# JunyiPeng00/wespeaker_hubert

Hardware: AMD Instinct MI355X
Metric: embeddings/sec on 5s 16kHz utts (higher is better)
Workload: dtype f32 (bf16x3 split MFMA, fp32 accumulate)

## Files before the change

wespeaker_hubert_amd/csrc/conv_gemm.hip:

```cpp
#include "gemm_common.h"

namespace wsp {

namespace {

constexpr int BK = 32;
constexpr int LDK = BK + 4;

template <int WM, int WN, int TM, int TN, int AMODE, bool UNI>
__global__ __launch_bounds__(256, 2) void conv_gemm_f32(const ConvGemmArgs p) {
  constexpr int BM = WM * TM * 32;
  constexpr int BN = WN * TN * 32;
  constexpr int AR = BM / 32;
  constexpr int BR = BN / 32;
  static_assert(WM * WN == 4, "4 waves");

  extern __shared__ __attribute__((aligned(16))) float smem[];
  float* As = smem;
  float* Bs = smem + 2 * BM * LDK;

  const int tid = threadIdx.x;
  const int lane = tid & 63;
  const int wave = tid >> 6;
  const int ntiles = p.N / BN;
  const int mtiles = (p.M + BM - 1) / BM;
  const int wg = xcd_remap(blockIdx.x, ntiles * mtiles);
  const int mt = wg / ntiles;
  const int nt = wg - mt * ntiles;
  const int m0 = mt * BM;
  const int n0 = nt * BN;

  const int srow = tid >> 3;
  const int c4 = (tid & 7) * 4;
  ALoader<AR, AMODE, UNI> al;
  al.init(p, m0, srow, 32, c4);
  if (p.gcols) al.a0 += (n0 / p.gcols) * p.gcin;
  const __amdgpu_buffer_rsrc_t rw = make_rsrc(p.w);
  int woff[BR];
#pragma unroll
  for (int i = 0; i < BR; ++i) woff[i] = ((n0 + srow + 32 * i) * p.Kp + c4) * 4;

  f32x4 ra[AR], rb[BR];

  auto load_tile = [&](int k0) {
#pragma unroll
    for (int i = 0; i < BR; ++i) rb[i] = bload4(rw, woff[i] + k0 * 4);
    al.load(k0, ra);
  };

  auto store_tile = [&](int buf) {
    float* a = As + buf * BM * LDK;
    float* b = Bs + buf * BN * LDK;
#pragma unroll
    for (int i = 0; i < AR; ++i)
      *reinterpret_cast<f32x4*>(a + (srow + 32 * i) * LDK + c4) = ra[i];
#pragma unroll
    for (int i = 0; i < BR; ++i)
      *reinterpret_cast<f32x4*>(b + (srow + 32 * i) * LDK + c4) = rb[i];
  };

  const int wm = wave / WN;
  const int wn = wave - wm * WN;
  const int r32 = lane & 31;
  const int h = lane >> 5;

  f32x16 acc[TM][TN];
#pragma unroll
  for (int i = 0; i < TM; ++i)
#pragma unroll
    for (int j = 0; j < TN; ++j)
#pragma unroll
      for (int r = 0; r < 16; ++r) acc[i][j][r] = 0.f;

  const int nk = p.Kp / BK;
  load_tile(0);
  store_tile(0);
  __syncthreads();

  for (int kt = 0; kt < nk; ++kt) {
    const int cur = kt & 1;
    if (kt + 1 < nk) load_tile((kt + 1) * BK);
    const float* a = As + cur * BM * LDK + (wm * TM * 32 + r32) * LDK + h * 16;
    const float* b = Bs + cur * BN * LDK + (wn * TN * 32 + r32) * LDK + h * 16;
#pragma unroll
    for (int q = 0; q < 4; ++q) {
      f32x4 af[TM], bf[TN];
#pragma unroll
      for (int i = 0; i < TM; ++i) af[i] = *reinterpret_cast<const f32x4*>(a + i * 32 * LDK + q * 4);
#pragma unroll
      for (int j = 0; j < TN; ++j) bf[j] = *reinterpret_cast<const f32x4*>(b + j * 32 * LDK + q * 4);
#pragma unroll
      for (int s = 0; s < 4; ++s)
#pragma unroll
        for (int i = 0; i < TM; ++i)
#pragma unroll
          for (int j = 0; j < TN; ++j)
            acc[i][j] = __builtin_amdgcn_mfma_f32_32x32x2f32(af[i][s], bf[j][s], acc[i][j], 0, 0, 0);
    }
    if (kt + 1 < nk) store_tile(cur ^ 1);
    __syncthreads();
  }

  gemm_epilogue<TM, TN>(p, acc, m0, n0, wm, wn, lane);
}

template <int WM, int WN, int TM, int TN, int AMODE, bool UNI>
void launch_k(const ConvGemmArgs& p, hipStream_t s) {
  constexpr int BM = WM * TM * 32, BN = WN * TN * 32;
  const int nwg = ((p.M + BM - 1) / BM) * (p.N / BN);
  const size_t lds = (size_t)2 * (BM + BN) * LDK * sizeof(float);
  hipLaunchKernelGGL((conv_gemm_f32<WM, WN, TM, TN, AMODE, UNI>), dim3(nwg), dim3(256), lds, s, p);
  WSP_HIP(hipGetLastError());
}

template <int WM, int WN, int TM, int TN>
void launch_tile(const ConvGemmArgs& p, hipStream_t s) {
  const bool uni = uniform_ktiles(p);
  if (p.amode == kAAdd) {
    if (uni) launch_k<WM, WN, TM, TN, kAAdd, true>(p, s);
    else launch_k<WM, WN, TM, TN, kAAdd, false>(p, s);
  } else {
    if (uni) launch_k<WM, WN, TM, TN, kACat, true>(p, s);
    else launch_k<WM, WN, TM, TN, kACat, false>(p, s);
  }
}

}

int conv_gemm_tile_for(int N) { return (N % 128 == 0) ? 0 : 1; }

void launch_conv_gemm(const ConvGemmArgs& args, hipStream_t s) {
  const ConvGemmArgs p = normalized(args);
  check_conv_args(p, "conv_gemm");
  WSP_CHECK(!p.colsum, "conv_gemm: column sums are a bf16x3-kernel epilogue");
  WSP_CHECK(!p.conv2d && p.N % 64 == 0, "conv_gemm (f32): 1-D convs with N % 64 == 0 only");
  WSP_CHECK(!p.gcols || p.gcols % 64 == 0, "conv_gemm (f32): grouped columns must be a multiple of 64");
  WSP_CHECK(!p.sc2d && !p.lnmode && !p.gate && !p.seam_h && !p.seam_out,
            "conv_gemm (f32): conv3 + shortcut, the LayerNorm fold, the gated A tail and the seam run on tile family 7");
  if (conv_gemm_tile_for(p.N) == 0 && !p.gcols)
    launch_tile<2, 2, 2, 2>(p, s);
  else
    launch_tile<4, 1, 1, 2>(p, s);
}

}
```

wespeaker_hubert_amd/csrc/conv_gemm_x3.hip:

```cpp
#include "conv_gemm_x3_impl.h"

namespace wsp {

int conv_gemm_x3_block_rows(const ConvGemmArgs& p, int variant) {
  if (p.N % 64 != 0 || (p.gcols && p.gcols % 64 != 0)) return 128;
  if (p.gcols || p.N % 128 != 0) return 128;
  return variant == 3 ? 128 : 256;
}

namespace {
__global__ __launch_bounds__(256) void colsum_mean_kernel(const double* __restrict__ part, int bm, int T, int N,
                                                          float* __restrict__ out, int ldo) {
  const int b = blockIdx.y;
  const int n = blockIdx.x * 256 + threadIdx.x;
  if (n >= N) return;
  const long r0 = (long)b * T, r1 = r0 + T;
  double v = 0.0;
  for (long mt = r0 / bm; mt * bm < r1; ++mt) {
    const int slot = (mt * bm) / T == b ? 0 : 1;
    v += part[((size_t)mt * 2 + slot) * N + n];
  }
  out[(long)b * ldo + n] = (float)(v / (double)T);
}
}

void launch_colsum_mean(const double* part, int block_rows, int T, int B, int N, float* out, int ldo,
                        hipStream_t s) {
  WSP_CHECK(block_rows > 0 && T >= block_rows && B > 0 && N > 0, "colsum_mean: bad shape");
  hipLaunchKernelGGL(colsum_mean_kernel, dim3((N + 255) / 256, B), dim3(256), 0, s, part, block_rows, T, N, out,
                     ldo);
  WSP_HIP(hipGetLastError());
}

bool conv_gemm_x3_gate_ok(const ConvGemmArgs& args, int variant) {
  return variant == 7 && args.gate && x3::g256_gate_supported(normalized(args));
}

bool conv_gemm_x3_seam_ok(const ConvGemmArgs& args, int variant) {
  return variant == 7 && args.seam_h && x3::seam_supported(normalized(args));
}

void launch_conv_gemm_x3(const ConvGemmArgs& args, const void* whi, const void* wlo, int variant,
                         hipStream_t s) {
  const ConvGemmArgs p = normalized(args);
  check_conv_args(p, "conv_gemm_x3");
  if (p.colsum) {
    const int bm = conv_gemm_x3_block_rows(p, variant);
    WSP_CHECK(!p.seg && !p.row_bias && !p.conv2d && p.T >= bm,
              "conv_gemm_x3: column sums need a uniform batch with T >= block rows and no row bias");
  }
  WSP_CHECK(p.Kp % 64 == 0, "conv_gemm_x3: packed K must be a multiple of 64");
  WSP_CHECK(variant >= 3 && variant <= 7, "conv_gemm_x3: tile family must be 3, 4, 5, 6 or 7");
  const __bf16* h = static_cast<const __bf16*>(whi);
  const __bf16* l = static_cast<const __bf16*>(wlo);
  x3::TileFn f;
  if (p.seam_h || p.seam_out) {
    WSP_CHECK(variant == 7 && x3::seam_supported(p),
              "conv_gemm_x3: the seam runs on tile family 7 only (conv_gemm_x3_seam_ok)");
    x3::t_seam(p, h, l, s);
    return;
  }
  WSP_CHECK(!p.lnmode || (variant == 7 && x3::g256_supported(p)),
            "conv_gemm_x3: the LayerNorm fold runs on tile family 7 only");
  WSP_CHECK(!p.sc2d || (variant == 7 && x3::g256_supported(p)),
            "conv_gemm_x3: conv3 + shortcut runs on tile family 7 only (N % 256 == 0, 16-B aligned operands)");
  WSP_CHECK(!p.gate || (variant == 7 && x3::g256_gate_supported(p)),
            "conv_gemm_x3: the gated A tail runs on tile family 7 only (conv_gemm_x3_gate_ok)");
  if (variant == 7 && x3::g256_supported(p)) {
    x3::t_g256(p, h, l, s);
    return;
  }
  if (variant == 7) variant = 6;
  if (p.N % 64 != 0 || (p.gcols && p.gcols % 64 != 0)) {
    f = x3::t_4x1_1x1;
  } else if (p.gcols) {
    f = variant >= 5 ? x3::t_8x1_1x2_sw : x3::t_4x1_1x2;
  } else if (p.N % 128 != 0) {
    f = x3::t_4x1_1x2;
  } else if (variant == 3) {
    f = x3::t_2x2_2x2_sw;
  } else if (variant == 4) {
    f = x3::t_4x2_2x2_sw;
  } else if (p.N % 256 == 0) {
    f = variant == 6 ? x3::t_4x2_2x4_mf16 : x3::t_4x2_2x4_sw1;
  } else {
    f = x3::t_4x2_2x2_sw;
  }
  f(p, h, l, s);
}

}
```

wespeaker_hubert_amd/csrc/conv_gemm_x3_g.h:

```cpp
#pragma once

#include "conv_gemm_x3_impl.h"

namespace wsp {
namespace {

typedef __attribute__((address_space(3))) void lds_void;
constexpr int kGA = 256 * 128, kGW = 256 * 64, kGStage = kGA + 2 * kGW;

__device__ __forceinline__ int g_aslot(int r, int c) { return r * 128 + ((c ^ ((r >> 1) & 5)) << 4); }

__device__ __forceinline__ void g_dma(__amdgpu_buffer_rsrc_t r, unsigned char* lds, int voff) {
  __builtin_amdgcn_raw_ptr_buffer_load_lds(r, (lds_void*)lds, 16, voff, 0, 0, 0);
}

constexpr int kGEpiLd = 132;
constexpr int kGEpiBytes = 8 * 32 * kGEpiLd * 4;
typedef unsigned u32x4 __attribute__((ext_vector_type(4)));

constexpr int kLnMaxParts = 8;
__device__ __forceinline__ void g_ln_row(const ConvGemmArgs& p, int row, float& mu, float& rstd) {
  const float* s = p.ln_in + (size_t)row * p.ln_parts * 2;
  float m = s[0], m2 = s[1];
#pragma unroll
  for (int k = 1; k < kLnMaxParts; ++k) {
    if (k < p.ln_parts) {
      const float d = s[2 * k] - m;
      m += d * (1.f / (float)(k + 1));
      m2 += s[2 * k + 1] + d * d * (128.f * (float)k / (float)(k + 1));
    }
  }
  mu = m;
  rstd = 1.f / sqrtf(m2 / (128.f * (float)p.ln_parts) + p.ln_eps);
}

template <int R>
__device__ __forceinline__ void g_ln_pieces(float (&m)[R], float (&m2)[R]) {
  float n = 4.f;
  auto merge = [&](int i, float mo, float m2o) {
    const float d = mo - m[i];
    m[i] = 0.5f * (m[i] + mo);
    m2[i] = (m2[i] + m2o) + d * d * (0.5f * n);
  };
#define WSP_DPP(v, ctrl) __builtin_bit_cast(float, __builtin_amdgcn_mov_dpp(__builtin_bit_cast(int, v), ctrl, 0xF, 0xF, false))
#pragma unroll
  for (int i = 0; i < R; ++i) merge(i, WSP_DPP(m[i], 0xB1), WSP_DPP(m2[i], 0xB1));
  n *= 2.f;
#pragma unroll
  for (int i = 0; i < R; ++i) merge(i, WSP_DPP(m[i], 0x4E), WSP_DPP(m2[i], 0x4E));
  n *= 2.f;
#pragma unroll
  for (int i = 0; i < R; ++i) merge(i, WSP_DPP(m[i], 0x141), WSP_DPP(m2[i], 0x141));
  n *= 2.f;
#pragma unroll
  for (int i = 0; i < R; ++i) merge(i, WSP_DPP(m[i], 0x140), WSP_DPP(m2[i], 0x140));
  n *= 2.f;
#undef WSP_DPP
#define WSP_BC15(v) \
  __builtin_bit_cast(float, __builtin_amdgcn_update_dpp(0, __builtin_bit_cast(int, v), 0x142, 0xA, 0xF, false))
#pragma unroll
  for (int i = 0; i < R; ++i) merge(i, WSP_BC15(m[i]), WSP_BC15(m2[i]));
#undef WSP_BC15
}

template <int ACT, bool RB, bool RES, int LNM = 0>
__device__ __forceinline__ void g_epilogue_rows(const ConvGemmArgs& p, f32x4 (&acc)[4][8], int m0, int n0, int wm,
                                                int wn, int wave, int lane, unsigned char* smem, float lmu = 0.f,
                                                float lrs = 1.f) {
  float* stg = reinterpret_cast<float*>(smem) + wave * 32 * kGEpiLd;
  const int c16 = lane & 15, q = lane >> 4;
  const int cl = 4 * (lane & 31);
  const int col = n0 + wn * 128 + cl;
  const f32x4 bv = p.bias ? *reinterpret_cast<const f32x4*>(p.bias + col) : f32x4{0.f, 0.f, 0.f, 0.f};
  const f32x4 sc = p.scale ? *reinterpret_cast<const f32x4*>(p.scale + col) : f32x4{1.f, 1.f, 1.f, 1.f};
  const f32x4 sh = p.scale ? *reinterpret_cast<const f32x4*>(p.shift + col) : f32x4{0.f, 0.f, 0.f, 0.f};
  f32x4 lcs{0.f, 0.f, 0.f, 0.f}, lg{1.f, 1.f, 1.f, 1.f}, lb{0.f, 0.f, 0.f, 0.f};
  if constexpr ((LNM & 2) != 0) lcs = *reinterpret_cast<const f32x4*>(p.ln_cs + col);
  if constexpr ((LNM & 4) != 0) {
    lg = *reinterpret_cast<const f32x4*>(p.ln_g + col);
    lb = *reinterpret_cast<const f32x4*>(p.ln_b + col);
  }
  const int lparts = p.N / 128, lpart = (n0 + wn * 128) / 128;
  const __amdgpu_buffer_rsrc_t ro = make_rsrc(p.out);
  const __amdgpu_buffer_rsrc_t rres = make_rsrc(RES ? p.res : p.out);
#pragma unroll
  for (int h = 0; h < 2; ++h) {
    float pm[(LNM & 1) ? 16 : 1], pm2[(LNM & 1) ? 16 : 1];
#pragma unroll
    for (int i2 = 0; i2 < 2; ++i2)
#pragma unroll
      for (int j = 0; j < 8; ++j)
#pragma unroll
        for (int r = 0; r < 4; ++r) stg[(i2 * 16 + 4 * q + r) * kGEpiLd + j * 16 + c16] = acc[2 * h + i2][j][r];
    asm volatile("s_waitcnt lgkmcnt(0)" ::: "memory");
#pragma unroll
    for (int u = 0; u < 16; ++u) {
      const int rl = 2 * u + (lane >> 5);
      const int row = m0 + wm * 64 + h * 32 + rl;
      const bool ok = row < p.M;
      const f32x4 x = *reinterpret_cast<const f32x4*>(stg + rl * kGEpiLd + cl);
      f32x4 rv{0.f, 0.f, 0.f, 0.f}, rb{0.f, 0.f, 0.f, 0.f};
      if constexpr (RES) rv = bload4(rres, ok ? (row * p.ldres + col) * 4 : kOOB);
      if constexpr (RB) {
        const int rowc = ok ? row : p.M - 1;
        const int ub = p.seg ? seg_of(p.seg, p.nseg, rowc) : rowc / p.T;
        rb = *reinterpret_cast<const f32x4*>(p.row_bias + (size_t)ub * p.N + col);
      }
      float mu = 0.f, rstd = 1.f;
      if constexpr ((LNM & 6) != 0) {
        auto rd = [](float v, int l) {
          return __builtin_bit_cast(float, __builtin_amdgcn_readlane(__builtin_bit_cast(int, v), l));
        };
        mu = lane < 32 ? rd(lmu, h * 32 + 2 * u) : rd(lmu, h * 32 + 2 * u + 1);
        rstd = lane < 32 ? rd(lrs, h * 32 + 2 * u) : rd(lrs, h * 32 + 2 * u + 1);
      }
      f32x4 y;
#pragma unroll
      for (int e = 0; e < 4; ++e) {
        float v;
        if constexpr ((LNM & 2) != 0) v = (x[e] - mu * lcs[e]) * rstd + bv[e];
        else v = x[e] + bv[e];
        if constexpr ((LNM & 4) != 0) v += (rv[e] - mu) * rstd * lg[e] + lb[e];
        else if constexpr (RES) v += rv[e];
        if constexpr (RB) v += rb[e];
        if constexpr (ACT == kActRelu) v = fmaxf(v, 0.f);
        else if constexpr (ACT == kActTanh) v = tanhf(v);
        else if constexpr (ACT == kActGelu) v = gelu_as(v);
        y[e] = v * sc[e] + sh[e];
      }
      __builtin_amdgcn_raw_buffer_store_b128(__builtin_bit_cast(u32x4, y), ro, ok ? (row * p.ldo + col) * 4 : kOOB, 0,
                                             0);
      if constexpr ((LNM & 1) != 0) {
        pm[u] = ((y[0] + y[1]) + (y[2] + y[3])) * 0.25f;
        float q2 = 0.f;
#pragma unroll
        for (int e = 0; e < 4; ++e) q2 += (y[e] - pm[u]) * (y[e] - pm[u]);
        pm2[u] = q2;
      }
    }
    if constexpr ((LNM & 1) != 0) {
      g_ln_pieces<16>(pm, pm2);
      if ((lane & 31) == 16) {
#pragma unroll
        for (int u = 0; u < 16; ++u) {
          const int row = m0 + wm * 64 + h * 32 + 2 * u + (lane >> 5);
          if (row < p.M) *reinterpret_cast<float2*>(p.ln_out + ((size_t)row * lparts + lpart) * 2) = float2{pm[u], pm2[u]};
        }
      }
    }
    asm volatile("s_waitcnt lgkmcnt(0)" ::: "memory");
  }
}

}
}
```

wespeaker_hubert_amd/csrc/conv_gemm_x3_impl.h:

```cpp
#pragma once

#include <type_traits>

#include "gemm_common.h"

namespace wsp {

namespace {

typedef __bf16 bf16x8 __attribute__((ext_vector_type(8)));
typedef __bf16 bf16x4 __attribute__((ext_vector_type(4)));

constexpr int BK = 32;

template <bool SWZ, int MF = 32>
struct Lds {
  static constexpr int ROWB = SWZ ? 64 : 80;
  static constexpr int SKEW = SWZ ? 0 : 64;
  __device__ __forceinline__ static int off(int row, int byte) {
    static_assert(MF == 32 || SWZ, "16x16 fragments need the swizzled rows");
    if constexpr (SWZ && MF == 16)
      return row * 64 + ((((byte >> 4) ^ (0x1320 >> (4 * ((row >> 2) & 3)))) & 3) << 4) + (byte & 15);
    else if constexpr (SWZ) return row * 64 + ((((byte >> 4) ^ (row >> 2)) & 3) << 4) + (byte & 15);
    else return row * 80 + byte;
  }
};

template <int WM, int WN, int TM, int TN, int AMODE, bool UNI, int ROLE, bool C2D = false, bool SWZ = false,
          int NSET = 2, int MF = 32>
__global__ __launch_bounds__(WM* WN * 64, 2) void conv_gemm_x3(const ConvGemmArgs p,
                                                               const __bf16* __restrict__ whi,
                                                               const __bf16* __restrict__ wlo) {
  using L = Lds<SWZ, MF>;
  static_assert(MF == 32 || NSET == 1, "16x16 MFMA: one-staging-set wide tiles only");
  constexpr int ROWB = L::ROWB;
  constexpr int NT = WM * WN * 64;
  constexpr int BM = WM * TM * 32;
  constexpr int BN = WN * TN * 32;
  constexpr int AR = BM * 8 / NT;
  constexpr int BR = BN * 8 / NT;
  constexpr int ROWS_A = NT / 8;
  constexpr int A_BYTES = BM * ROWB;
  constexpr int B_BYTES = BN * ROWB;
  constexpr int B_LO = B_BYTES + L::SKEW;
  constexpr int STAGE = 2 * A_BYTES + B_LO + B_BYTES;
  static_assert(AR >= 1 && BR >= 1, "tile too small for the thread count");
  static_assert(BN * 4 % 64 == 0, "a W image must be a whole number of wave loads");

  extern __shared__ __attribute__((aligned(16))) unsigned char smem[];

  const int tid = threadIdx.x;
  const int lane = tid & 63;
  const int wave = tid >> 6;
  const int ntiles = p.N / BN;
  const int mtiles = (p.M + BM - 1) / BM;
  const int wg = xcd_remap(blockIdx.x, ntiles * mtiles);
  const int mt = wg / ntiles;
  const int nt = wg - mt * ntiles;
  const int m0 = mt * BM;
  const int n0 = nt * BN;

  const int srow = tid >> 3;
  const int c4 = (tid & 7) * 4;
  std::conditional_t<C2D, ALoader2D<AR>, ALoader<AR, AMODE, UNI>> al;
  al.init(p, m0, srow, ROWS_A, c4);
  if (p.gcols) al.a0 += (n0 / p.gcols) * p.gcin;
  const __amdgpu_buffer_rsrc_t rwhi = make_rsrc(whi);
  const __amdgpu_buffer_rsrc_t rwlo = make_rsrc(wlo);
  int boff[BR], bls[BR];
  bool bimg[BR];
#pragma unroll
  for (int i = 0; i < BR; ++i) {
    const int q = tid + NT * i;
    const int img = __builtin_amdgcn_readfirstlane(q / (BN * 4));
    const int qq = q - img * BN * 4;
    const int row = qq >> 2, part = qq & 3;
    bimg[i] = img != 0;
    boff[i] = ((n0 + row) * p.Kp + part * 8) * 2;
    bls[i] = L::off(row, part * 16) + (img ? B_LO : 0);
  }

  f32x4 ra0[AR], ra1[AR];
  bf16x8 rb0[BR], rb1[BR];

  auto load_tile = [&](f32x4 (&ra)[AR], bf16x8 (&rb)[BR], int k0, bool live) {
#pragma unroll
    for (int i = 0; i < BR; ++i) {
      const int o = live ? boff[i] + k0 * 2 : kOOB;
      rb[i] = __builtin_bit_cast(bf16x8, __builtin_amdgcn_raw_buffer_load_b128(bimg[i] ? rwlo : rwhi, o, 0, 0));
    }
    al.load(k0, ra, live);
  };

  auto store_tile = [&](const f32x4 (&ra)[AR], const bf16x8 (&rb)[BR], int buf) {
    unsigned char* st = smem + buf * STAGE;
#pragma unroll
    for (int i = 0; i < AR; ++i) {
      bf16x4 hi, lo;
#pragma unroll
      for (int e = 0; e < 4; ++e) {
        const float x = ra[i][e];
        const __bf16 hh = (__bf16)x;
        hi[e] = hh;
        lo[e] = (__bf16)(x - (float)hh);
      }
      const int off = L::off(srow + ROWS_A * i, c4 * 2);
      *reinterpret_cast<bf16x4*>(st + off) = hi;
      *reinterpret_cast<bf16x4*>(st + A_BYTES + off) = lo;
    }
#pragma unroll
    for (int i = 0; i < BR; ++i) *reinterpret_cast<bf16x8*>(st + 2 * A_BYTES + bls[i]) = rb[i];
  };

  const int wm = wave / WN;
  const int wn = wave - wm * WN;
  const int r32 = lane & 31;
  const int h = lane >> 5;

  f32x16 acc[TM][TN];
#pragma unroll
  for (int i = 0; i < TM; ++i)
#pragma unroll
    for (int j = 0; j < TN; ++j)
#pragma unroll
      for (int r = 0; r < 16; ++r) acc[i][j][r] = 0.f;

  auto mma_step = [&](int buf, int s) {
    const unsigned char* st = smem + buf * STAGE;
    const unsigned char* a_hi = st + L::off(wm * TM * 32 + r32, h * 16 + s * 32);
    const unsigned char* a_lo = a_hi + A_BYTES;
    const unsigned char* b_hi = st + 2 * A_BYTES + L::off(wn * TN * 32 + r32, h * 16 + s * 32);
    const unsigned char* b_lo = b_hi + B_LO;
    bf16x8 ah[TM], al_[TM], bh[TN], bl[TN];
#pragma unroll
    for (int i = 0; i < TM; ++i) {
      ah[i] = *reinterpret_cast<const bf16x8*>(a_hi + i * 32 * ROWB);
      al_[i] = *reinterpret_cast<const bf16x8*>(a_lo + i * 32 * ROWB);
    }
#pragma unroll
    for (int j = 0; j < TN; ++j) {
      bh[j] = *reinterpret_cast<const bf16x8*>(b_hi + j * 32 * ROWB);
      bl[j] = *reinterpret_cast<const bf16x8*>(b_lo + j * 32 * ROWB);
    }
#pragma unroll
    for (int i = 0; i < TM; ++i)
#pragma unroll
      for (int j = 0; j < TN; ++j) {
        acc[i][j] = __builtin_amdgcn_mfma_f32_32x32x16_bf16(al_[i], bh[j], acc[i][j], 0, 0, 0);
        acc[i][j] = __builtin_amdgcn_mfma_f32_32x32x16_bf16(ah[i], bl[j], acc[i][j], 0, 0, 0);
        acc[i][j] = __builtin_amdgcn_mfma_f32_32x32x16_bf16(ah[i], bh[j], acc[i][j], 0, 0, 0);
      }
  };

  const int nk = p.Kp / BK;
  if constexpr (MF == 16) {
    const int r16 = lane & 15, qk = lane >> 4;
    f32x4 acc16[2 * TM][2 * TN];
#pragma unroll
    for (int i = 0; i < 2 * TM; ++i)
#pragma unroll
      for (int j = 0; j < 2 * TN; ++j) acc16[i][j] = f32x4{0.f, 0.f, 0.f, 0.f};
    bf16x8 fah[TM], fal[TM], fbh[TN], fbl[TN];
    auto rdA = [&](const unsigned char* st, int ih) {
#pragma unroll
      for (int i = 0; i < TM; ++i) {
        const int o = L::off(wm * TM * 32 + (ih * TM + i) * 16 + r16, qk * 16);
        fah[i] = *reinterpret_cast<const bf16x8*>(st + o);
        fal[i] = *reinterpret_cast<const bf16x8*>(st + A_BYTES + o);
      }
    };
    auto rdB = [&](const unsigned char* st, int jh) {
#pragma unroll
      for (int j = 0; j < TN; ++j) {
        const int o = L::off(wn * TN * 32 + (jh * TN + j) * 16 + r16, qk * 16);
        fbh[j] = *reinterpret_cast<const bf16x8*>(st + 2 * A_BYTES + o);
        fbl[j] = *reinterpret_cast<const bf16x8*>(st + 2 * A_BYTES + B_LO + o);
      }
    };
    auto mm = [&](int ih, int jh) {
#pragma unroll
      for (int i = 0; i < TM; ++i)
#pragma unroll
        for (int j = 0; j < TN; ++j) {
          f32x4& c = acc16[ih * TM + i][jh * TN + j];
          c = __builtin_amdgcn_mfma_f32_16x16x32_bf16(fal[i], fbh[j], c, 0, 0, 0);
          c = __builtin_amdgcn_mfma_f32_16x16x32_bf16(fah[i], fbl[j], c, 0, 0, 0);
          c = __builtin_amdgcn_mfma_f32_16x16x32_bf16(fah[i], fbh[j], c, 0, 0, 0);
        }
    };
    load_tile(ra0, rb0, 0, true);
    store_tile(ra0, rb0, 0);
    load_tile(ra0, rb0, BK, true);
    __syncthreads();
    for (int kt = 0; kt < nk; ++kt) {
      const int buf = kt & 1;
      const unsigned char* st = smem + buf * STAGE;
      rdA(st, 0);
      rdB(st, 0);
      mm(0, 0);
      rdB(st, 1);
      mm(0, 1);
      store_tile(ra0, rb0, buf ^ 1);
      load_tile(ra0, rb0, (kt + 2) * BK, kt + 2 < nk);
      rdA(st, 1);
      mm(1, 1);
      rdB(st, 0);
      mm(1, 0);
      __syncthreads();
    }
    gemm_epilogue16<2 * TM, 2 * TN, WM, WN>(p, acc16, m0, n0, wm, wn, lane, smem);
    return;
  } else if constexpr (NSET == 1) {
    load_tile(ra0, rb0, 0, true);
    store_tile(ra0, rb0, 0);
    load_tile(ra0, rb0, BK, true);
    __syncthreads();
    for (int kt = 0; kt < nk; ++kt) {
      const int buf = kt & 1;
      mma_step(buf, 0);
      store_tile(ra0, rb0, buf ^ 1);
      load_tile(ra0, rb0, (kt + 2) * BK, kt + 2 < nk);
      mma_step(buf, 1);
      __syncthreads();
    }
    gemm_epilogue<TM, TN, WM, WN>(p, acc, m0, n0, wm, wn, lane, smem);
    return;
  }
  load_tile(ra0, rb0, 0, true);
  load_tile(ra1, rb1, BK, true);
  store_tile(ra0, rb0, 0);
  __syncthreads();

  if constexpr (ROLE == 2) {
    for (int kt = 0; kt < nk - 2; kt += 2) {
      load_tile(ra0, rb0, (kt + 2) * BK, true);
      mma_step(0, 0);
      store_tile(ra1, rb1, 1);
      mma_step(0, 1);
      __syncthreads();
      load_tile(ra1, rb1, (kt + 3) * BK, true);
      mma_step(1, 0);
      store_tile(ra0, rb0, 0);
      mma_step(1, 1);
      __syncthreads();
    }
    float rv[TM][TN][16];
    load_residual_tiles<TM, TN>(p, rv, m0, n0, wm, wn, lane);
    mma_step(0, 0);
    store_tile(ra1, rb1, 1);
    mma_step(0, 1);
    __syncthreads();
    mma_step(1, 0);
    mma_step(1, 1);
    gemm_epilogue_res_pre<TM, TN>(p, acc, m0, n0, wm, wn, lane, rv);
    return;
  }

  for (int kt = 0; kt < nk; kt += 2) {
    load_tile(ra0, rb0, (kt + 2) * BK, kt + 2 < nk);
    mma_step(0, 0);
    store_tile(ra1, rb1, 1);
    mma_step(0, 1);
    __syncthreads();
    load_tile(ra1, rb1, (kt + 3) * BK, kt + 3 < nk);
    mma_step(1, 0);
    store_tile(ra0, rb0, 0);
    mma_step(1, 1);
    __syncthreads();
  }

  gemm_epilogue<TM, TN, WM, WN>(p, acc, m0, n0, wm, wn, lane, smem);
}

template <int WM, int WN, int TM, int TN, int AMODE, bool UNI, int ROLE, bool C2D, bool SWZ, int NSET, int MF = 32>
void launch_x3_k(const ConvGemmArgs& p, const __bf16* whi, const __bf16* wlo, hipStream_t s) {
  constexpr int BM = WM * TM * 32, BN = WN * TN * 32, NT = WM * WN * 64;
  constexpr int ROWB = Lds<SWZ>::ROWB;
  const int nwg = ((p.M + BM - 1) / BM) * (p.N / BN);
  const size_t lds = (size_t)2 * (2 * BM * ROWB + 2 * BN * ROWB + Lds<SWZ>::SKEW);
  hipLaunchKernelGGL((conv_gemm_x3<WM, WN, TM, TN, AMODE, UNI, ROLE, C2D, SWZ, NSET, MF>), dim3(nwg), dim3(NT), lds,
                     s, p, whi, wlo);
  WSP_HIP(hipGetLastError());
}

template <int WM, int WN, int TM, int TN, bool SWZ = false, int NSET = 2, int MF = 32>
void launch_x3_tile(const ConvGemmArgs& p, const __bf16* whi, const __bf16* wlo, hipStream_t s) {
  if constexpr (MF == 32) {
    if (p.conv2d) {
      launch_x3_k<WM, WN, TM, TN, kACat, true, 0, true, SWZ, NSET, MF>(p, whi, wlo, s);
      return;
    }
  }
  const bool uni = uniform_ktiles(p);
  if (MF == 32 && p.amode == kAAdd) {
    if constexpr (MF == 32) {
      if (uni)
        launch_x3_k<WM, WN, TM, TN, kAAdd, true, 0, false, SWZ, NSET, MF>(p, whi, wlo, s);
      else
        launch_x3_k<WM, WN, TM, TN, kAAdd, false, 0, false, SWZ, NSET, MF>(p, whi, wlo, s);
    }
  } else if (!uni) {
    launch_x3_k<WM, WN, TM, TN, kACat, false, 0, false, SWZ, NSET, MF>(p, whi, wlo, s);
  } else if (p.role == 1) {
    launch_x3_k<WM, WN, TM, TN, kACat, true, 1, false, SWZ, NSET, MF>(p, whi, wlo, s);
  } else if constexpr (NSET == 2 && TM * TN <= 4) {
    if (p.res && p.role == 2)
      launch_x3_k<WM, WN, TM, TN, kACat, true, 2, false, SWZ, NSET>(p, whi, wlo, s);
    else
      launch_x3_k<WM, WN, TM, TN, kACat, true, 0, false, SWZ, NSET>(p, whi, wlo, s);
  } else {
    launch_x3_k<WM, WN, TM, TN, kACat, true, 0, false, SWZ, NSET, MF>(p, whi, wlo, s);
  }
}

}

namespace x3 {
using TileFn = void (*)(const ConvGemmArgs&, const __bf16*, const __bf16*, hipStream_t);
void t_4x1_1x1(const ConvGemmArgs&, const __bf16*, const __bf16*, hipStream_t);
void t_4x1_1x2(const ConvGemmArgs&, const __bf16*, const __bf16*, hipStream_t);
void t_8x1_1x2_sw(const ConvGemmArgs&, const __bf16*, const __bf16*, hipStream_t);
void t_2x2_2x2_sw(const ConvGemmArgs&, const __bf16*, const __bf16*, hipStream_t);
void t_4x2_2x2_sw(const ConvGemmArgs&, const __bf16*, const __bf16*, hipStream_t);
void t_4x2_2x4_sw1(const ConvGemmArgs&, const __bf16*, const __bf16*, hipStream_t);
void t_4x2_2x4_mf16(const ConvGemmArgs&, const __bf16*, const __bf16*, hipStream_t);
bool g256_supported(const ConvGemmArgs&);
bool g256_gate_supported(const ConvGemmArgs&);
void t_g256(const ConvGemmArgs&, const __bf16*, const __bf16*, hipStream_t);
bool seam_supported(const ConvGemmArgs&);
void t_seam(const ConvGemmArgs&, const __bf16*, const __bf16*, hipStream_t, bool balanced = true);
}

}
```

wespeaker_hubert_amd/csrc/conv_gemm_x3_t6.hip:

```cpp
#include "conv_gemm_x3_g.h"

namespace wsp {
namespace {

constexpr int kGCsLd = 68;
constexpr int kGCsBytes = 8 * 64 * kGCsLd * 4;
template <int ACT>
__device__ __forceinline__ void g_epilogue_cs(const ConvGemmArgs& p, f32x4 (&acc)[4][8], int m0, int n0, int wm,
                                              int wn, int wave, int lane, unsigned char* smem) {
  float* stg = reinterpret_cast<float*>(smem) + wave * 64 * kGCsLd;
  const int c16 = lane & 15, q = lane >> 4;
  const int cl = 4 * c16;
  const __amdgpu_buffer_rsrc_t ro = make_rsrc(p.out);
  const int nb = min((m0 / p.T + 1) * p.T, p.M) - m0, mb = p.M - m0;
  unsigned side0 = 0, side1 = 0;
#pragma unroll
  for (int k = 0; k < 16; ++k) {
    const int rr = wm * 64 + (k >> 2) * 16 + 4 * q + (k & 3);
    side0 |= (rr < nb ? 1u : 0u) << k;
    side1 |= (rr >= nb && rr < mb ? 1u : 0u) << k;
  }
  double rs[8][2];
#pragma unroll
  for (int pp = 0; pp < 2; ++pp) {
#pragma unroll
    for (int i = 0; i < 4; ++i)
#pragma unroll
      for (int jj = 0; jj < 4; ++jj)
#pragma unroll
        for (int r = 0; r < 4; ++r) stg[(16 * i + 4 * q + r) * kGCsLd + 16 * jj + c16] = acc[i][4 * pp + jj][r];
    asm volatile("s_waitcnt lgkmcnt(0)" ::: "memory");
    const int col = n0 + wn * 128 + 64 * pp + cl;
    const f32x4 bv = p.bias ? *reinterpret_cast<const f32x4*>(p.bias + col) : f32x4{0.f, 0.f, 0.f, 0.f};
    const f32x4 sc = p.scale ? *reinterpret_cast<const f32x4*>(p.scale + col) : f32x4{1.f, 1.f, 1.f, 1.f};
    const f32x4 sh = p.scale ? *reinterpret_cast<const f32x4*>(p.shift + col) : f32x4{0.f, 0.f, 0.f, 0.f};
#pragma unroll
    for (int u = 0; u < 16; ++u) {
      const int rl = 4 * u + q;
      const int row = m0 + wm * 64 + rl;
      float* sp = stg + rl * kGCsLd + cl;
      const f32x4 x = *reinterpret_cast<const f32x4*>(sp);
      f32x4 y;
#pragma unroll
      for (int e = 0; e < 4; ++e) {
        float v = x[e] + bv[e];
        if constexpr (ACT == kActRelu) v = fmaxf(v, 0.f);
        else if constexpr (ACT == kActTanh) v = tanhf(v);
        else if constexpr (ACT == kActGelu) v = gelu_as(v);
        y[e] = v * sc[e] + sh[e];
      }
      __builtin_amdgcn_raw_buffer_store_b128(__builtin_bit_cast(u32x4, y), ro,
                                             row < p.M ? (row * p.ldo + col) * 4 : kOOB, 0, 0);
      *reinterpret_cast<f32x4*>(sp) = y;
    }
    asm volatile("s_waitcnt lgkmcnt(0)" ::: "memory");
#pragma unroll
    for (int jj = 0; jj < 4; ++jj) {
      double c0 = 0.0, c1 = 0.0;
#pragma unroll
      for (int k = 0; k < 16; ++k) {
        const double yd = (double)stg[((k >> 2) * 16 + 4 * q + (k & 3)) * kGCsLd + 16 * jj + c16];
        c0 += (side0 >> k) & 1 ? yd : 0.0;
        c1 += (side1 >> k) & 1 ? yd : 0.0;
      }
      double v0 = c0 + __shfl_xor(c0, 16);
      v0 += __shfl_xor(v0, 32);
      double v1 = c1 + __shfl_xor(c1, 16);
      v1 += __shfl_xor(v1, 32);
      rs[4 * pp + jj][0] = v0;
      rs[4 * pp + jj][1] = v1;
      __builtin_amdgcn_sched_barrier(0);
    }
    asm volatile("s_waitcnt lgkmcnt(0)" ::: "memory");
  }
  __syncthreads();
  constexpr int BN = 256;
  double* red = reinterpret_cast<double*>(smem);
  if (lane < 16) {
#pragma unroll
    for (int j = 0; j < 8; ++j)
#pragma unroll
      for (int u = 0; u < 2; ++u) red[(wm * 2 + u) * BN + (wn * 8 + j) * 16 + lane] = rs[j][u];
  }
  __syncthreads();
  const int tid = threadIdx.x;
  if (tid < 2 * BN) {
    const int u = tid / BN, c = tid - u * BN;
    double v = 0.0;
#pragma unroll
    for (int w = 0; w < 4; ++w) v += red[(w * 2 + u) * BN + c];
    p.colsum[((size_t)(m0 / 256) * 2 + u) * p.N + n0 + c] = v;
  }
}

template <int AM, bool CSK, int LNM = 0>
__global__ __launch_bounds__(512, 1) void conv_gemm_g(const ConvGemmArgs p, const __bf16* __restrict__ whi,
                                                      const __bf16* __restrict__ wlo) {
  using L = Lds<true, 16>;
  constexpr bool DENSE = AM == 1 || AM == 3 || AM == 4;
  constexpr bool GATE = AM == 4;
  static_assert(!GATE || (!CSK && LNM == 0), "the gated instance: plain epilogues only");
  extern __shared__ __attribute__((aligned(16))) unsigned char smem[];
  const int tid = threadIdx.x;
  const int lane = tid & 63;
  const int wave = tid >> 6;
  const int ntiles = p.N / 256;
  const int mtiles = (p.M + 255) / 256;
  const int wg = xcd_remap(blockIdx.x, ntiles * mtiles);
  const int mt = wg / ntiles;
  const int nt = wg - mt * ntiles;
  const int m0 = mt * 256;
  const int n0 = nt * 256;

  const int ac0 = 4 * ((lane & 7) ^ ((lane >> 4) & 1)), ac1 = ac0 ^ 16;
  int a_r[4], a_t[DENSE ? 1 : 4], a_l[DENSE ? 1 : 4], a_s[AM == 3 ? 4 : 1];
#pragma unroll
  for (int i = 0; i < 4; ++i) {
    const int m = m0 + (4 * wave + i) * 8 + (lane >> 3);
    if constexpr (DENSE) {
      a_r[i] = m < p.M ? m : -1;
      if constexpr (AM == 3) {
        const int fto = p.Fo * p.To;
        const int b = m / fto, fo = (m - b * fto) / p.To, to = m - b * fto - fo * p.To;
        a_s[i] = m < p.M ? (b * p.Fi + fo * p.stride) * p.Ti + to * p.stride : -1;
      }
    } else if (p.seg) {
      const int mm = m < p.M ? m : p.M - 1;
      const int b = seg_of(p.seg, p.nseg, mm);
      const int t = (mm - p.seg[b]) * p.stride;
      const int* is = p.iseg ? p.iseg : p.seg;
      a_r[i] = is[b] + t;
      a_t[i] = (m < p.M) ? t : -0x40000000;
      a_l[i] = is[b + 1] - is[b];
    } else {
      const int b = m / p.T;
      const int t = (m - b * p.T) * p.stride;
      a_r[i] = b * p.Ti + t;
      a_t[i] = (m < p.M) ? t : -0x40000000;
      a_l[i] = p.Ti;
    }
  }
  int woff[2];
#pragma unroll
  for (int i = 0; i < 2; ++i) {
    const int row = (2 * wave + i) * 16 + (lane >> 2);
    const int c = (lane & 3) ^ ((0x1320 >> (4 * ((row >> 2) & 3))) & 3);
    woff[i] = ((n0 + row) * p.Kp + 8 * c) * 2;
  }
  const __amdgpu_buffer_rsrc_t rwh = make_rsrc(whi);
  const __amdgpu_buffer_rsrc_t rwl = make_rsrc(wlo);
  const int nk = p.Kp / BK;
  int jt = 0, ct = 0;
  auto dma = [&](int kt, int buf) {
    unsigned char* st = smem + buf * kGStage;
    const int off = jt * p.dil - p.pad;
    const float* base = p.a[0];
    int ld = p.lda[0], cl = ct;
    if (ct >= p.cseg[2]) {
      base = p.a[2];
      ld = p.lda[2];
      cl = ct - p.cseg[2];
    } else if (ct >= p.cseg[1]) {
      base = p.a[1];
      ld = p.lda[1];
      cl = ct - p.cseg[1];
    }
    const __amdgpu_buffer_rsrc_t ra = make_rsrc(base);
#pragma unroll
    for (int i = 0; i < 4; ++i) {
      if constexpr (DENSE) {
        const int ar = AM == 3 && ct >= p.cseg[1] ? a_s[i] : a_r[i];
        g_dma(ra, st + (4 * wave + i) * 1024, ar >= 0 ? (ar * ld + cl + (i & 1 ? ac1 : ac0)) * 4 : kOOB);
      } else if constexpr (AM == 2) {
        const int k = kt * BK + (i & 1 ? ac1 : ac0);
        const int tap = k / p.cin;
        const int offk = tap * p.dil - p.pad;
        const int tt = a_t[i] + offk;
        const bool ok = k < p.K && tt >= 0 && tt < a_l[i];
        g_dma(ra, st + (4 * wave + i) * 1024, ok ? ((a_r[i] + offk) * ld + k - tap * p.cin) * 4 : kOOB);
      } else {
        const int tt = a_t[i] + off;
        const bool ok = tt >= 0 && tt < a_l[i];
        g_dma(ra, st + (4 * wave + i) * 1024, ok ? ((a_r[i] + off) * ld + cl + (i & 1 ? ac1 : ac0)) * 4 : kOOB);
      }
    }
#pragma unroll
    for (int i = 0; i < 2; ++i) {
      const int o = woff[i] + kt * 64;
      g_dma(rwh, st + kGA + (2 * wave + i) * 1024, o);
      g_dma(rwl, st + kGA + kGW + (2 * wave + i) * 1024, o);
    }
    ct += 32;
    if (ct >= p.cin) {
      ct -= p.cin;
      ++jt;
    }
  };

  const int wm = wave >> 1, wn = wave & 1;
  const int r16 = lane & 15, qk = lane >> 4;
  f32x4 acc[4][8];
#pragma unroll
  for (int i = 0; i < 4; ++i)
#pragma unroll
    for (int j = 0; j < 8; ++j) acc[i][j] = f32x4{0.f, 0.f, 0.f, 0.f};
  bf16x8 ah[2], al[2], bh[4], bl[4];
  const int g_nb = GATE ? min((m0 / p.T + 1) * p.T, p.M) - m0 : 0;
  const int g_slot = GATE ? (p.K - p.gate_k0) * 4 : 0;
  auto rdA = [&](auto gated, const unsigned char* st, int ih, const unsigned char* gp = nullptr) {
#pragma clang fp contract(off)
#pragma unroll
    for (int i = 0; i < 2; ++i) {
      const int r = wm * 64 + (ih * 2 + i) * 16 + r16;
      f32x4 x0 = *reinterpret_cast<const f32x4*>(st + g_aslot(r, 2 * qk));
      f32x4 x1 = *reinterpret_cast<const f32x4*>(st + g_aslot(r, 2 * qk + 1));
      if constexpr (decltype(gated)::value) {
        const unsigned char* gr = gp + (r >= g_nb ? g_slot : 0);
        x0 = x0 * *reinterpret_cast<const f32x4*>(gr);
        x1 = x1 * *reinterpret_cast<const f32x4*>(gr + 16);
      }
#pragma unroll
      for (int e = 0; e < 4; ++e) {
        const __bf16 h0 = (__bf16)x0[e], h1 = (__bf16)x1[e];
        ah[i][e] = h0;
        ah[i][4 + e] = h1;
        al[i][e] = (__bf16)(x0[e] - (float)h0);
        al[i][4 + e] = (__bf16)(x1[e] - (float)h1);
      }
    }
  };
  auto rdB = [&](const unsigned char* st, int jh) {
#pragma unroll
    for (int j = 0; j < 4; ++j) {
      const int o = L::off(wn * 128 + (jh * 4 + j) * 16 + r16, qk * 16);
      bh[j] = *reinterpret_cast<const bf16x8*>(st + kGA + o);
      bl[j] = *reinterpret_cast<const bf16x8*>(st + kGA + kGW + o);
    }
  };
  auto mm = [&](int ih, int jh) {
#pragma unroll
    for (int i = 0; i < 2; ++i)
#pragma unroll
      for (int j = 0; j < 4; ++j) {
        f32x4& c = acc[ih * 2 + i][jh * 4 + j];
        c = __builtin_amdgcn_mfma_f32_16x16x32_bf16(al[i], bh[j], c, 0, 0, 0);
        c = __builtin_amdgcn_mfma_f32_16x16x32_bf16(ah[i], bl[j], c, 0, 0, 0);
        c = __builtin_amdgcn_mfma_f32_16x16x32_bf16(ah[i], bh[j], c, 0, 0, 0);
      }
  };

  float lmu = 0.f, lrs = 1.f;
  if constexpr ((LNM & 6) != 0) g_ln_row(p, min(m0 + wm * 64 + lane, p.M - 1), lmu, lrs);
  if constexpr (GATE) {
    const int ppu = g_slot >> 10, b0 = m0 / p.T;
    const __amdgpu_buffer_rsrc_t rg = make_rsrc(p.gate);
#pragma unroll
    for (int i = 0; i < 4; ++i) {
      const int q = 8 * i + wave;
      if (q >= 2 * ppu) break;
      const int u = q >= ppu ? 1 : 0;
      const bool ok = (b0 + u) * p.T < p.M;
      g_dma(rg, smem + 2 * kGStage + q * 1024, ok ? ((b0 + u) * p.ldg + (q - u * ppu) * 256 + lane * 4) * 4 : kOOB);
    }
  }
  dma(0, 0);
  dma(1, 1);
  asm volatile("s_waitcnt vmcnt(8)" ::: "memory");
  __builtin_amdgcn_s_barrier();
  auto ktile = [&](auto gated, int kt) {
    const int buf = kt & 1;
    const unsigned char* st = smem + buf * kGStage;
    const unsigned char* gp =
        decltype(gated)::value ? smem + 2 * kGStage + (kt * BK - p.gate_k0 + 8 * qk) * 4 : nullptr;
    rdA(gated, st, 0, gp);
    rdB(st, 0);
    mm(0, 0);
    rdB(st, 1);
    mm(0, 1);
    rdA(gated, st, 1, gp);
    mm(1, 1);
    rdB(st, 0);
    mm(1, 0);
    asm volatile("s_waitcnt vmcnt(0) lgkmcnt(0)" ::: "memory");
    __builtin_amdgcn_s_barrier();
    __builtin_amdgcn_sched_barrier(0);
    if (kt + 2 < nk) dma(kt + 2, buf);
  };
  const int ktg = GATE ? p.gate_k0 / BK : nk;
  for (int kt = 0; kt < ktg; ++kt) ktile(std::false_type{}, kt);
  if constexpr (GATE)
    for (int kt = ktg; kt < nk; ++kt) ktile(std::true_type{}, kt);
#define WSP_GEPI(RB, RES)                                                                                   \
  switch (p.act) {                                                                                         \
    case kActRelu: g_epilogue_rows<kActRelu, RB, RES>(p, acc, m0, n0, wm, wn, wave, lane, smem); break;    \
    case kActTanh: g_epilogue_rows<kActTanh, RB, RES>(p, acc, m0, n0, wm, wn, wave, lane, smem); break;    \
    case kActGelu: g_epilogue_rows<kActGelu, RB, RES>(p, acc, m0, n0, wm, wn, wave, lane, smem); break;    \
    default: g_epilogue_rows<kActNone, RB, RES>(p, acc, m0, n0, wm, wn, wave, lane, smem); break;          \
  }
  if constexpr (LNM != 0) {
    if constexpr ((LNM & 5) != 0)
      g_epilogue_rows<kActNone, false, true, LNM>(p, acc, m0, n0, wm, wn, wave, lane, smem, lmu, lrs);
    else if (p.act == kActGelu)
      g_epilogue_rows<kActGelu, false, false, LNM>(p, acc, m0, n0, wm, wn, wave, lane, smem, lmu, lrs);
    else
      g_epilogue_rows<kActNone, false, false, LNM>(p, acc, m0, n0, wm, wn, wave, lane, smem, lmu, lrs);
  } else if constexpr (CSK) {
    switch (p.act) {
      case kActRelu: g_epilogue_cs<kActRelu>(p, acc, m0, n0, wm, wn, wave, lane, smem); break;
      case kActTanh: g_epilogue_cs<kActTanh>(p, acc, m0, n0, wm, wn, wave, lane, smem); break;
      case kActGelu: g_epilogue_cs<kActGelu>(p, acc, m0, n0, wm, wn, wave, lane, smem); break;
      default: g_epilogue_cs<kActNone>(p, acc, m0, n0, wm, wn, wave, lane, smem); break;
    }
  } else if (p.res) {
    WSP_GEPI(false, true)
  } else if (p.row_bias) {
    WSP_GEPI(true, false)
  } else {
    WSP_GEPI(false, false)
  }
#undef WSP_GEPI
}

}

namespace x3 {

bool g256_supported(const ConvGemmArgs& p) {
  auto a16 = [](const void* q) { return (reinterpret_cast<uintptr_t>(q) & 15) == 0; };
  const bool aligned = a16(p.out) && p.ldo % 4 == 0 && a16(p.bias) && a16(p.scale) && a16(p.shift) &&
                       a16(p.row_bias) && a16(p.res) && (!p.res || p.ldres % 4 == 0);
  return aligned && p.N % 256 == 0 && !p.conv2d && !p.gcols && p.amode == kACat &&
         (uniform_ktiles(p) || (p.cseg[1] >= p.cin && !p.colsum)) &&
         (!p.sc2d || (uniform_ktiles(p) && !p.colsum && !p.lnmode && !p.row_bias));
}

bool g256_gate_supported(const ConvGemmArgs& p) {
  if (!p.gate || !g256_supported(p) || !uniform_ktiles(p)) return false;
  const bool dense = p.taps == 1 && p.pad == 0 && p.stride == 1 && !p.iseg && !p.seg && p.Ti == p.T;
  const int gk = p.K - p.gate_k0;
  return dense && p.T >= 256 && p.M % p.T == 0 && !p.colsum && !p.lnmode && !p.sc2d && p.K == p.Kp &&
         p.gate_k0 >= 0 && p.gate_k0 % 32 == 0 && gk > 0 && gk % 128 == 0 && gk <= 4096 && p.ldg >= gk &&
         p.ldg % 4 == 0 && (reinterpret_cast<uintptr_t>(p.gate) & 15) == 0 &&
         (long long)(p.M / p.T) * p.ldg * 4 < (long long)kOOB;
}

void t_g256(const ConvGemmArgs& p, const __bf16* h, const __bf16* l, hipStream_t s) {
  const int nwg = ((p.M + 255) / 256) * (p.N / 256);
  constexpr int lds0 = 2 * kGStage > kGEpiBytes ? 2 * kGStage : kGEpiBytes;
  constexpr int lds = lds0 > kGCsBytes ? lds0 : kGCsBytes;
  const bool dense = p.taps == 1 && p.pad == 0 && p.stride == 1 && !p.iseg && (p.seg || p.Ti == p.T);
  const int am = !uniform_ktiles(p) ? 2 : dense ? 1 : 0;
  if (p.gate) {
    WSP_CHECK(g256_gate_supported(p), "conv_gemm_x3: the gated A tail needs a dense 1x1 GEMM over a uniform batch");
    const int ldsg = std::max(lds, 2 * kGStage + 2 * (p.K - p.gate_k0) * 4);
    hipLaunchKernelGGL((conv_gemm_g<4, false>), dim3(nwg), dim3(512), ldsg, s, p, h, l);
    WSP_HIP(hipGetLastError());
    return;
  }
  if (p.sc2d) {
    hipLaunchKernelGGL((conv_gemm_g<3, false>), dim3(nwg), dim3(512), lds, s, p, h, l);
    WSP_HIP(hipGetLastError());
    return;
  }
  if (p.lnmode) {
    WSP_CHECK(am == 1 && !p.colsum && !p.row_bias && !p.scale && p.N % 128 == 0 &&
                  ((p.lnmode & 1) == 0 || (p.ln_out && p.res && p.act == kActNone)) &&
                  ((p.lnmode & 6) == 0 || (p.ln_in && p.ln_parts >= 1 && p.ln_parts <= kLnMaxParts)) && ((p.lnmode & 2) == 0 || (p.ln_cs && !p.res)) &&
                  (p.lnmode != 2 || p.act == kActNone || p.act == kActGelu) &&
                  ((p.lnmode & 4) == 0 || (p.ln_g && p.ln_b && p.res && p.act == kActNone)),
              "conv_gemm_x3: LayerNorm fold needs a dense 1x1 GEMM and its operands (fold: no activation or GELU)");
    switch (p.lnmode) {
      case 1: hipLaunchKernelGGL((conv_gemm_g<1, false, 1>), dim3(nwg), dim3(512), lds, s, p, h, l); break;
      case 2: hipLaunchKernelGGL((conv_gemm_g<1, false, 2>), dim3(nwg), dim3(512), lds, s, p, h, l); break;
      case 4: hipLaunchKernelGGL((conv_gemm_g<1, false, 4>), dim3(nwg), dim3(512), lds, s, p, h, l); break;
      case 5: hipLaunchKernelGGL((conv_gemm_g<1, false, 5>), dim3(nwg), dim3(512), lds, s, p, h, l); break;
      default: WSP_CHECK(false, "conv_gemm_x3: lnmode must be 1, 2, 4 or 5");
    }
    WSP_HIP(hipGetLastError());
    return;
  }
  if (p.colsum && am == 1)
    hipLaunchKernelGGL((conv_gemm_g<1, true>), dim3(nwg), dim3(512), lds, s, p, h, l);
  else if (p.colsum && am == 0)
    hipLaunchKernelGGL((conv_gemm_g<0, true>), dim3(nwg), dim3(512), lds, s, p, h, l);
  else if (am == 1)
    hipLaunchKernelGGL((conv_gemm_g<1, false>), dim3(nwg), dim3(512), lds, s, p, h, l);
  else if (am == 0)
    hipLaunchKernelGGL((conv_gemm_g<0, false>), dim3(nwg), dim3(512), lds, s, p, h, l);
  else
    hipLaunchKernelGGL((conv_gemm_g<2, false>), dim3(nwg), dim3(512), lds, s, p, h, l);
  WSP_HIP(hipGetLastError());
}

}
}
```

wespeaker_hubert_amd/csrc/conv_gemm_x3_t7.hip:

```cpp
#include "conv_gemm_x3_g.h"

namespace wsp {
namespace {

constexpr int kSPlane = 256 * 64;
constexpr int kSStage = 4 * kSPlane;

template <bool BAL>
__global__ __launch_bounds__(512, 1) void conv_gemm_seam(const ConvGemmArgs p, const __bf16* __restrict__ whi,
                                                         const __bf16* __restrict__ wlo) {
  using L = Lds<true, 16>;
  extern __shared__ __attribute__((aligned(16))) unsigned char smem[];
  const int tid = threadIdx.x;
  const int lane = tid & 63;
  const int wave = tid >> 6;
  const int ntiles = p.N / 256;
  const int mtiles = (p.M + 255) / 256;
  const int wg = xcd_remap(blockIdx.x, ntiles * mtiles);
  const int mt = wg / ntiles;
  const int nt = wg - mt * ntiles;
  const int m0 = mt * 256;
  const int n0 = nt * 256;
  const int nk = p.K / BK;

  const int srow = tid >> 3, c8 = tid & 7;
  const __amdgpu_buffer_rsrc_t rx = make_rsrc(p.a[0]);
  const __amdgpu_buffer_rsrc_t rh = make_rsrc(p.seam_h);
  const __amdgpu_buffer_rsrc_t rs = make_rsrc(p.seam_out);
  const int g_nb = min((m0 / p.T + 1) * p.T, p.M) - m0;
  int a_r[4];
  bool a_u[4];
#pragma unroll
  for (int i = 0; i < 4; ++i) {
    const int r = srow + 64 * i;
    a_r[i] = m0 + r < p.M ? m0 + r : -1;
    a_u[i] = r >= g_nb;
  }
  f32x4 vx[4], vh[4];
  auto load_a = [&](int kt, int i0) {
    const int kc = kt * BK + 4 * c8;
#pragma unroll
    for (int i = i0; i < i0 + 2; ++i) {
      const bool ok = kt < nk && a_r[i] >= 0;
      vx[i] = bload4(rx, ok ? (a_r[i] * p.lda[0] + kc) * 4 : kOOB);
      vh[i] = bload4(rh, ok ? (a_r[i] * p.ld_seam_h + kc) * 4 : kOOB);
    }
  };
  int woff[2];
#pragma unroll
  for (int i = 0; i < 2; ++i) {
    const int row = (2 * wave + i) * 16 + (lane >> 2);
    const int c = (lane & 3) ^ ((0x1320 >> (4 * ((row >> 2) & 3))) & 3);
    woff[i] = ((n0 + row) * p.Kp + 8 * c) * 2;
  }
  const __amdgpu_buffer_rsrc_t rwh = make_rsrc(whi);
  const __amdgpu_buffer_rsrc_t rwl = make_rsrc(wlo);
  auto dma_w = [&](int kt, int buf) {
    unsigned char* st = smem + buf * kSStage;
#pragma unroll
    for (int i = 0; i < 2; ++i) {
      const int o = kt < nk ? woff[i] + kt * 64 : kOOB;
      g_dma(rwh, st + 2 * kSPlane + (2 * wave + i) * 1024, o);
      g_dma(rwl, st + 3 * kSPlane + (2 * wave + i) * 1024, o);
    }
  };
  unsigned char* const gl = smem + 2 * kSStage;
  {
    const __amdgpu_buffer_rsrc_t rg = make_rsrc(p.gate);
    const int b0 = m0 / p.T, nch = p.K / 4;
    for (int q = tid; q < 2 * nch; q += 512) {
      const int u = q >= nch ? 1 : 0;
      const bool ok = (b0 + u) * p.T < p.M;
      *reinterpret_cast<f32x4*>(gl + q * 16) = bload4(rg, ok ? ((b0 + u) * p.ldg + 4 * (q - u * nch)) * 4 : kOOB);
    }
  }

  int own = BAL ? nt : 0;
  auto store_rows = [&](int kt, int buf, int i0) {
#pragma clang fp contract(off)
    unsigned char* st = smem + buf * kSStage;
    const int kc = kt * BK + 4 * c8;
    const int kg = kt < nk ? kc : 4 * c8;
    const f32x4 g0 = *reinterpret_cast<const f32x4*>(gl + kg * 4);
    const f32x4 g1 = *reinterpret_cast<const f32x4*>(gl + (p.K + kg) * 4);
    const bool mine = (BAL || nt == 0) && kt == own && kt < nk;
    if (mine && i0 == 2) own += BAL ? ntiles : 1;
#pragma unroll
    for (int i = i0; i < i0 + 2; ++i) {
      const f32x4 g = a_u[i] ? g1 : g0;
      f32x4 v;
      bf16x4 hi, lo;
#pragma unroll
      for (int e = 0; e < 4; ++e) {
        v[e] = __builtin_fmaf(vh[i][e], g[e], vx[i][e]);
        const __bf16 hh = (__bf16)v[e];
        hi[e] = hh;
        lo[e] = (__bf16)(v[e] - (float)hh);
      }
      __builtin_amdgcn_raw_buffer_store_b128(__builtin_bit_cast(u32x4, v), rs,
                                             mine && a_r[i] >= 0 ? (a_r[i] * p.ld_seam_out + kc) * 4 : kOOB, 0, 0);
      const int off = L::off(srow + 64 * i, c8 * 8);
      *reinterpret_cast<bf16x4*>(st + off) = hi;
      *reinterpret_cast<bf16x4*>(st + kSPlane + off) = lo;
    }
  };

  const int wm = wave >> 1, wn = wave & 1;
  const int r16 = lane & 15, qk = lane >> 4;
  f32x4 acc[4][8];
#pragma unroll
  for (int i = 0; i < 4; ++i)
#pragma unroll
    for (int j = 0; j < 8; ++j) acc[i][j] = f32x4{0.f, 0.f, 0.f, 0.f};
  bf16x8 ah[2], al[2], bh[4], bl[4];
  auto rdA = [&](const unsigned char* st, int ih) {
#pragma unroll
    for (int i = 0; i < 2; ++i) {
      const int o = L::off(wm * 64 + (ih * 2 + i) * 16 + r16, qk * 16);
      ah[i] = *reinterpret_cast<const bf16x8*>(st + o);
      al[i] = *reinterpret_cast<const bf16x8*>(st + kSPlane + o);
    }
  };
  auto rdB = [&](const unsigned char* st, int jh) {
#pragma unroll
    for (int j = 0; j < 4; ++j) {
      const int o = L::off(wn * 128 + (jh * 4 + j) * 16 + r16, qk * 16);
      bh[j] = *reinterpret_cast<const bf16x8*>(st + 2 * kSPlane + o);
      bl[j] = *reinterpret_cast<const bf16x8*>(st + 3 * kSPlane + o);
    }
  };
  auto mm = [&](int ih, int jh) {
#pragma unroll
    for (int i = 0; i < 2; ++i)
#pragma unroll
      for (int j = 0; j < 4; ++j) {
        f32x4& c = acc[ih * 2 + i][jh * 4 + j];
        c = __builtin_amdgcn_mfma_f32_16x16x32_bf16(al[i], bh[j], c, 0, 0, 0);
        c = __builtin_amdgcn_mfma_f32_16x16x32_bf16(ah[i], bl[j], c, 0, 0, 0);
        c = __builtin_amdgcn_mfma_f32_16x16x32_bf16(ah[i], bh[j], c, 0, 0, 0);
      }
  };

  auto interleave = [] {
#pragma unroll
    for (int z = 0; z < 48; ++z) {
      __builtin_amdgcn_sched_group_barrier(0x008, 1, 0);
      __builtin_amdgcn_sched_group_barrier(0x002, 2, 0);
    }
  };
  load_a(0, 0);
  load_a(0, 2);
  dma_w(0, 0);
  asm volatile("s_waitcnt vmcnt(0) lgkmcnt(0)" ::: "memory");
  __builtin_amdgcn_s_barrier();
  __builtin_amdgcn_sched_barrier(0);
  store_rows(0, 0, 0);
  store_rows(0, 0, 2);
  load_a(1, 0);
  load_a(1, 2);
  asm volatile("s_waitcnt lgkmcnt(0)" ::: "memory");
  __builtin_amdgcn_s_barrier();
  __builtin_amdgcn_sched_barrier(0);
  for (int kt = 0; kt < nk; ++kt) {
    const int buf = kt & 1;
    const unsigned char* st = smem + buf * kSStage;
    dma_w(kt + 1, buf ^ 1);
    __builtin_amdgcn_sched_barrier(0);
    rdA(st, 0);
    rdB(st, 0);
    mm(0, 0);
    rdB(st, 1);
    mm(0, 1);
    store_rows(kt + 1, buf ^ 1, 0);
    load_a(kt + 2, 0);
    interleave();
    __builtin_amdgcn_sched_barrier(0);
    rdA(st, 1);
    mm(1, 1);
    rdB(st, 0);
    mm(1, 0);
    store_rows(kt + 1, buf ^ 1, 2);
    load_a(kt + 2, 2);
    interleave();
    asm volatile("s_waitcnt vmcnt(12) lgkmcnt(0)" ::: "memory");
    __builtin_amdgcn_s_barrier();
    __builtin_amdgcn_sched_barrier(0);
  }
  switch (p.act) {
    case kActRelu: g_epilogue_rows<kActRelu, false, false>(p, acc, m0, n0, wm, wn, wave, lane, smem); break;
    case kActTanh: g_epilogue_rows<kActTanh, false, false>(p, acc, m0, n0, wm, wn, wave, lane, smem); break;
    case kActGelu: g_epilogue_rows<kActGelu, false, false>(p, acc, m0, n0, wm, wn, wave, lane, smem); break;
    default: g_epilogue_rows<kActNone, false, false>(p, acc, m0, n0, wm, wn, wave, lane, smem); break;
  }
}

}

namespace x3 {

bool seam_supported(const ConvGemmArgs& p) {
  if (!p.seam_h || !p.seam_out || !p.gate || !g256_supported(p) || !uniform_ktiles(p)) return false;
  auto a16 = [](const void* q) { return (reinterpret_cast<uintptr_t>(q) & 15) == 0; };
  const bool dense = p.taps == 1 && p.pad == 0 && p.stride == 1 && !p.iseg && !p.seg && p.Ti == p.T && p.cseg[1] == p.cin;
  const bool plain = !p.colsum && !p.lnmode && !p.sc2d && !p.res && !p.row_bias;
  const bool lds = p.K == p.Kp && p.K % 64 == 0 && p.K <= 4096;
  const bool ops = a16(p.a[0]) && a16(p.seam_h) && a16(p.seam_out) && a16(p.gate) && p.gate_k0 == 0 && p.ldg >= p.K &&
                   p.ldg % 4 == 0 && p.lda[0] >= p.K && p.ld_seam_h >= p.K && p.ld_seam_h % 4 == 0 &&
                   p.ld_seam_out >= p.K && p.ld_seam_out % 4 == 0;
  if (!dense || !plain || !lds || !ops || p.T < 256 || p.M % p.T != 0) return false;
  const long long lim = kOOB;
  return (long long)(p.M / p.T) * p.ldg * 4 < lim && (long long)p.M * p.ld_seam_h * 4 < lim &&
         (long long)p.M * p.ld_seam_out * 4 < lim;
}

void t_seam(const ConvGemmArgs& p, const __bf16* h, const __bf16* l, hipStream_t s, bool balanced) {
  WSP_CHECK(seam_supported(p), "conv_gemm_x3: the seam needs a dense 1x1 GEMM over a uniform batch with T >= 256");
  const int nwg = ((p.M + 255) / 256) * (p.N / 256);
  const int lds = std::max(2 * kSStage + 2 * p.K * 4, kGEpiBytes);
  if (balanced)
    hipLaunchKernelGGL((conv_gemm_seam<true>), dim3(nwg), dim3(512), lds, s, p, h, l);
  else
    hipLaunchKernelGGL((conv_gemm_seam<false>), dim3(nwg), dim3(512), lds, s, p, h, l);
  WSP_HIP(hipGetLastError());
}

}
}
```

wespeaker_hubert_amd/csrc/ecapa_model.cpp:

```cpp
#include "astp_fused.h"
#include "model_impl.h"
#include "res2_chain.h"
#include "xi_pool.h"

namespace wsp {

namespace {
struct Ecapa final : Model::Impl {
  using Impl::Impl;
  int C = 512;
  bool glob = false;
  bool xi = false;
  ConvW layer1;
  struct Block {
    ConvW c1, c3, res2[7];
    LinW se1, se2;
    void* r2w = nullptr;
    float *r2b = nullptr, *r2s = nullptr, *r2t = nullptr;
  } blk[3];
  ConvW conv, pool1, pool2;
  ConvW conv_g;
  void* pool2_frag = nullptr;
  LinW pool1_ctx;
  float *prior_mean = nullptr, *prior_logprec = nullptr;
  LinW head;
  int pooled_dim() const { return xi ? 1536 : 3072; }

  void build_params() override;
  void pack_res2(Block& b, const std::string& p, int w);
  void finalize() override;
  int chunk(int B, int T) const;
  size_t ws_floats(int B, int T) const override;
  void forward(const float* feats, int B, int T, float* embed, float* ws, hipStream_t s) override;
  void forward_chunk(const float* feats, int B, int T, float* embed, float* ws, hipStream_t s,
                     const int* seg = nullptr, int M_seg = 0);
  int min_frames() const override { return xi ? 1 : 2; }
  bool has_segments() const override { return true; }
  size_t ws_floats_segments(int B, int M) const override;
  void forward_segments(const float* feats, int B, const int* seg, int M, float* embed, float* ws,
                        hipStream_t s) override {
    forward_chunk(feats, B, 1, embed, ws, s, seg, M);
  }
};
}

Model::Impl* make_ecapa(const std::string& arch, int feat_dim, int embed_dim, bool emb_bn, bool two_emb) {
  const bool xi = arch == "XI_VEC_ECAPA_TDNN_c512" || arch == "XI_VEC_ECAPA_TDNN_c1024";
  if (!xi && arch != "ECAPA_TDNN_c512" && arch != "ECAPA_TDNN_GLOB_c512" && arch != "ECAPA_TDNN_c1024" &&
      arch != "ECAPA_TDNN_GLOB_c1024")
    return nullptr;
  WSP_CHECK(!(xi && two_emb), "XI_VEC_ECAPA_TDNN has no two_emb_layer");
  WSP_CHECK(feat_dim > 0 && feat_dim % 4 == 0, "ECAPA feat_dim must be a positive multiple of 4");
  WSP_CHECK(embed_dim > 0, "embed_dim must be positive");
  Ecapa* m = new Ecapa(arch, feat_dim, embed_dim, emb_bn, two_emb);
  m->opt.x3_variant = 7;
  m->C = (arch.find("c1024") != std::string::npos) ? 1024 : 512;
  m->glob = arch.find("GLOB") != std::string::npos;
  m->xi = xi;
  return m;
}

void Ecapa::build_params() {
  const int64_t C = this->C, w = C / 8;
  add("layer1.conv.weight", {C, feat_dim, 5});
  add("layer1.conv.bias", {C});
  add_bn("layer1.bn", C);
  for (int li = 2; li <= 4; ++li) {
    const std::string p = "layer" + std::to_string(li) + ".se_res2block";
    add(p + ".0.conv.weight", {C, C, 1});
    add(p + ".0.conv.bias", {C});
    add_bn(p + ".0.bn", C);
    for (int i = 0; i < 7; ++i) {
      add(p + ".1.convs." + std::to_string(i) + ".weight", {w, w, 3});
      add(p + ".1.convs." + std::to_string(i) + ".bias", {w});
    }
    for (int i = 0; i < 7; ++i) add_bn(p + ".1.bns." + std::to_string(i), w);
    add(p + ".2.conv.weight", {C, C, 1});
    add(p + ".2.conv.bias", {C});
    add_bn(p + ".2.bn", C);
    add(p + ".3.linear1.weight", {128, C});
    add(p + ".3.linear1.bias", {128});
    add(p + ".3.linear2.weight", {C, 128});
    add(p + ".3.linear2.bias", {C});
  }
  add("conv.weight", {1536, 3 * C, 1});
  add("conv.bias", {1536});
  if (xi) {
    add("pool.prior_mean", {1, 1536});
    add("pool.prior_logprec", {1, 1536});
    add("pool.lin1_relu_bn.0.weight", {256, 1536, 1});
    add("pool.lin1_relu_bn.0.bias", {256});
    add_bn("pool.lin1_relu_bn.2", 256);
    add("pool.lin2.weight", {1536, 256, 1});
    add("pool.lin2.bias", {1536});
  } else {
    add("pool.linear1.weight", {128, glob ? 4608 : 1536, 1});
    add("pool.linear1.bias", {128});
    add("pool.linear2.weight", {1536, 128, 1});
    add("pool.linear2.bias", {1536});
  }
  add_bn("bn", pooled_dim());
  add("linear.weight", {embed_dim, pooled_dim()});
  add("linear.bias", {embed_dim});
  if (emb_bn) add_bn("bn2", embed_dim);
}

void Ecapa::pack_res2(Block& b, const std::string& p, int w) {
  const std::vector<float>* W[7];
  std::vector<float> bias((size_t)7 * w), sc((size_t)7 * w), sh((size_t)7 * w);
  for (int i = 0; i < 7; ++i) {
    const std::string ci = p + ".1.convs." + std::to_string(i);
    W[i] = &P(ci + ".weight");
    const auto& bb = P(ci + ".bias");
    std::vector<double> s, t;
    bn_affine(p + ".1.bns." + std::to_string(i), s, t);
    for (int n = 0; n < w; ++n) {
      bias[(size_t)i * w + n] = bb[n];
      sc[(size_t)i * w + n] = (float)s[n];
      sh[(size_t)i * w + n] = (float)t[n];
    }
  }
  b.r2w = dev.upload_u16(pack::frag_res2(W, w));
  b.r2b = dev.upload(bias);
  b.r2s = dev.upload(sc);
  b.r2t = dev.upload(sh);
}

void Ecapa::finalize() {
  const int w = C / 8;
  layer1 = pack_conv(P("layer1.conv.weight"), C, feat_dim, 5, P("layer1.conv.bias").data(), "layer1.bn");
  for (int li = 0; li < 3; ++li) {
    const std::string p = "layer" + std::to_string(li + 2) + ".se_res2block";
    Block& b = blk[li];
    b.c1 = pack_conv(P(p + ".0.conv.weight"), C, C, 1, P(p + ".0.conv.bias").data(), p + ".0.bn");
    for (int i = 0; i < 7; ++i) {
      const std::string ci = p + ".1.convs." + std::to_string(i);
      b.res2[i] = pack_conv(P(ci + ".weight"), w, w, 3, P(ci + ".bias").data(), p + ".1.bns." + std::to_string(i));
    }
    if (res2_chain_supported(w, li + 2)) pack_res2(b, p, w);
    b.c3 = pack_conv(P(p + ".2.conv.weight"), C, C, 1, P(p + ".2.conv.bias").data(), p + ".2.bn");
    b.se1 = pack_lin(P(p + ".3.linear1.weight").data(), 128, C, C, P(p + ".3.linear1.bias").data());
    b.se2 = pack_lin(P(p + ".3.linear2.weight").data(), C, 128, 128, P(p + ".3.linear2.bias").data());
  }
  conv = pack_conv(P("conv.weight"), 1536, 3 * C, 1, P("conv.bias").data(), "");
  {
    std::vector<float> wg = P("conv.weight");
    for (int n = 0; n < 1536; ++n)
      for (int c = 0; c < C; ++c) {
        float* r = wg.data() + (size_t)n * 3 * C;
        r[C + c] = (float)((double)r[C + c] + (double)r[2 * C + c]);
      }
    conv_g = pack_conv(wg, 1536, 3 * C, 1, P("conv.bias").data(), "");
  }
  if (xi) {
    pool1 = pack_conv(P("pool.lin1_relu_bn.0.weight"), 256, 1536, 1, P("pool.lin1_relu_bn.0.bias").data(),
                      "pool.lin1_relu_bn.2");
    pool2 = pack_conv(P("pool.lin2.weight"), 1536, 256, 1, P("pool.lin2.bias").data(), "");
    prior_mean = dev.upload(P("pool.prior_mean"));
    prior_logprec = dev.upload(P("pool.prior_logprec"));
  } else {
    const auto& l1 = P("pool.linear1.weight");
    const int l1k = glob ? 4608 : 1536;
    std::vector<float> wx((size_t)128 * 1536);
    for (int n = 0; n < 128; ++n)
      for (int k = 0; k < 1536; ++k) wx[(size_t)n * 1536 + k] = l1[(size_t)n * l1k + k];
    pool1 = pack_conv(wx, 128, 1536, 1, P("pool.linear1.bias").data(), "");
    if (glob) {
      pool1_ctx = pack_lin(l1.data() + 1536, 128, 3072, l1k, P("pool.linear1.bias").data());
    }
    pool2 = pack_conv(P("pool.linear2.weight"), 1536, 128, 1, P("pool.linear2.bias").data(), "");
    pool2_frag = pack_frag(P("pool.linear2.weight"), 1536, 128);
  }
  {
    std::vector<double> s, t;
    bn_affine("bn", s, t);
    const auto& W = P("linear.weight");
    const auto& bb = P("linear.bias");
    const int D = embed_dim;
    std::vector<double> s2(D, 1.0), t2(D, 0.0);
    if (emb_bn) bn_affine("bn2", s2, t2);
    const int K = pooled_dim();
    std::vector<float> wf((size_t)D * K), bf(D);
    for (int n = 0; n < D; ++n) {
      double acc = bb[n];
      for (int k = 0; k < K; ++k) {
        const double wv = W[(size_t)n * K + k];
        wf[(size_t)n * K + k] = (float)(s2[n] * wv * s[k]);
        acc += wv * t[k];
      }
      bf[n] = (float)(s2[n] * acc + t2[n]);
    }
    head = pack_lin(wf.data(), D, K, K, bf.data());
  }
}

int Ecapa::chunk(int B, int T) const {
  return chunk_for(B, (size_t)T * std::max(C, 1536) * sizeof(float));
}

namespace {
struct EcapaWs {
  float *x[5], *h1, *h2, *h3, *gmean, *ghid, *gate, *xp, *att, *logit, *gstats, *rowb, *pooled;
  double* sesum;
  size_t floats;
};
EcapaWs ecapa_ws(size_t C, size_t B, size_t M, float* base, bool xi) {
  WsCursor c{base};
  EcapaWs w;
  w.x[0] = nullptr;
  for (int i = 1; i <= 4; ++i) w.x[i] = c.take(M * C);
  w.h1 = c.take(M * C);
  w.h2 = c.take(M * C);
  w.h3 = c.take(M * C);
  w.gmean = c.take(B * C);
  w.ghid = c.take(B * 128);
  w.gate = c.take(B * C);
  w.xp = c.take(M * 1536);
  w.att = c.take(M * (xi ? 256 : 128));
  w.logit = c.take(M * 1536);
  w.gstats = c.take(B * 3072);
  w.rowb = c.take(B * 128);
  w.pooled = c.take(B * 3072);
  w.sesum = reinterpret_cast<double*>(c.take(((M + 127) / 128) * 2 * C * 2));
  w.floats = c.off;
  return w;
}
}

size_t Ecapa::ws_floats(int B, int T) const {
  const size_t bc = chunk(B, T);
  return ecapa_ws(C, bc, bc * T, nullptr, xi).floats;
}

size_t Ecapa::ws_floats_segments(int B, int M) const { return ecapa_ws(C, B, M, nullptr, xi).floats; }

void Ecapa::forward(const float* feats, int B, int T, float* embed, float* ws, hipStream_t s) {
  const int bc = chunk(B, T);
  for (int c0 = 0; c0 < B; c0 += bc)
    forward_chunk(feats + (size_t)c0 * T * feat_dim, std::min(bc, B - c0), T, embed + (size_t)c0 * embed_dim, ws, s);
}

void Ecapa::forward_chunk(const float* feats, int B, int T, float* embed, float* ws, hipStream_t s,
                          const int* seg, int M_seg) {
  const int M = seg ? M_seg : B * T, w = C / 8;
  const EcapaWs W = ecapa_ws(C, B, M, ws, xi);
  float* const* x = W.x;
  float *h1 = W.h1, *h2 = W.h2, *h3 = W.h3, *xp = W.xp;
  const int se_bm = opt.precision == 1 ? conv_gemm_x3_block_rows(ConvGemmArgs{.N = C}, opt.x3_variant) : 0;
  const bool se_fused = opt.precision == 1 && !seg && T >= se_bm;
  auto gemm3 = [&](const char* tag, ConvGemmArgs& g, const ConvW& cw, int dil, int pad, float* out, int ldo) {
    g.lda[0] = g.lda[1] = g.lda[2] = C;
    fill(g, cw, M, T, dil, pad, out, ldo, kActRelu, nullptr, true, seg, B);
    run(tag, 2.0 * M * cw.N * cw.K, s, [&] { launch(g, cw, s); });
  };

  ConvGemmArgs gcat{};
  gcat.amode = kACat;
  gcat.a[0] = x[2];
  gcat.a[1] = x[3];
  gcat.a[2] = x[4];
  gcat.cseg[1] = C;
  gcat.cseg[2] = 2 * C;
  gcat.cseg[3] = 3 * C;
  gcat.lda[0] = gcat.lda[1] = gcat.lda[2] = C;
  const ConvW& wcat = opt.cat_gate ? conv_g : conv;
  bool fold = false;
  if (opt.cat_gate && opt.gate_fold && opt.precision == 1) {
    ConvGemmArgs g = gcat;
    g.a[2] = h3;
    g.gate = W.gate;
    g.ldg = C;
    g.gate_k0 = 2 * C;
    fill(g, wcat, M, T, 1, 0, xp, 1536, kActRelu, nullptr, true, seg, B);
    fold = conv_gemm_x3_gate_ok(g, opt.x3_variant);
    if (fold) gcat = g;
  }

  gemm("layer1", layer1, feats, feat_dim, x[1], C, M, T, 1, 2, kActRelu, s, seg, B);
  ConvGemmArgs gseam{};
  bool seam = false;
  for (int li = 0; li < 3; ++li) {
    const Block& b = blk[li];
    const int dil = li + 2;
    const float* xin = x[li + 1];
    if (seam) {
      run("se.scale", 0, s, [&] {
        run("seam", 0, s, [&] { run("conv1x1_CxC", 2.0 * M * C * C, s, [&] { launch(gseam, b.c1, s); }); });
      });
      seam = false;
    } else {
      gemm("conv1x1_CxC", b.c1, xin, C, h1, C, M, T, 1, 0, kActRelu, s, seg, B, nullptr, true, 1);
    }
    if (opt.precision == 1 && opt.res2_fused && b.r2w) {
      Res2Args r{};
      r.x = h1;
      r.out = h2;
      r.ldx = r.ldo = C;
      r.M = M;
      r.T = T;
      r.dil = dil;
      r.variant = w == 128 ? opt.res2_variant : std::min(opt.res2_variant, 3);
      r.rout = res2_chain_rout(dil, r.variant, M);
      r.seg = seg;
      r.nseg = B;
      r.w = b.r2w;
      r.bias = b.r2b;
      r.scale = b.r2s;
      r.shift = b.r2t;
      run("res2_k3", 7 * 2.0 * M * w * 3 * w, s, [&] { launch_res2_chain(r, w, s); });
    } else {
      for (int i = 0; i < 7; ++i) {
        ConvGemmArgs g{};
        g.amode = i == 0 ? kACat : kAAdd;
        if (i == 0) {
          one_operand(g, h1, C, w);
        } else {
          g.a[0] = h1 + i * w;
          g.a[1] = h2 + (i - 1) * w;
          g.a[2] = h1;
        }
        gemm3("res2_k3", g, b.res2[i], dil, dil, h2 + i * w, C);
      }
    }
    {
      ConvGemmArgs g{};
      g.amode = kACat;
      g.a[0] = h2;
      g.a[1] = h1 + 7 * w;
      g.a[2] = h1;
      g.cseg[1] = 7 * w;
      g.cseg[2] = g.cseg[3] = C;
      g.role = 1;
      if (se_fused) g.colsum = W.sesum;
      gemm3("conv1x1_CxC", g, b.c3, 1, 0, h3, C);
    }
    run("se", 0, s, [&] {
      if (se_fused) launch_colsum_mean(W.sesum, se_bm, T, B, C, W.gmean, C, s);
      else launch_frame_stats(h3, C, B, T, C, W.gmean, C, 0, 0, s, seg);
      launch_small_linear({W.gmean, C, b.se1.wt, b.se1.bias, W.ghid, 128, B, C, 128, 1}, s);
      launch_small_linear({W.ghid, 128, b.se2.wt, b.se2.bias, W.gate, C, B, 128, C, 3}, s);
    });
    if (li == 2 && fold) continue;
    if (li < 2 && opt.seam_fold && opt.precision == 1) {
      ConvGemmArgs g{};
      one_operand(g, xin, C, C);
      g.role = 1;
      g.seam_h = h3;
      g.ld_seam_h = C;
      g.gate = W.gate;
      g.ldg = C;
      g.seam_out = x[li + 2];
      g.ld_seam_out = C;
      fill(g, blk[li + 1].c1, M, T, 1, 0, h1, C, kActRelu, nullptr, true, seg, B);
      seam = conv_gemm_x3_seam_ok(g, opt.x3_variant);
      if (seam) {
        gseam = g;
        continue;
      }
    }
    run("se.scale", 0, s, [&] {
      launch_residual_scale(opt.cat_gate && li == 2 ? nullptr : xin, h3, W.gate, x[li + 2], B, T, C, s, seg, M);
    });
  }
  gemm3("conv_cat", gcat, wcat, 1, 0, xp, 1536);
  if (glob) {
    run("glob_ctx", 0, s, [&] {
      launch_frame_stats(xp, 1536, B, T, 1536, W.gstats, 3072, 1, 1536, s, seg);
      launch_small_linear({W.gstats, 3072, pool1_ctx.wt, pool1_ctx.bias, W.rowb, 128, B, 3072, 128, 0}, s);
    });
  }
  if (xi) {
    gemm("xi_lin1", pool1, xp, 1536, W.att, 256, M, T, 1, 0, kActRelu, s, seg, B);
    gemm("xi_lin2", pool2, W.att, 256, W.logit, 1536, M, T, 1, 0, kActNone, s, seg, B);
    const XiPoolArgs a{W.logit, 1536, xp, 1536, prior_mean, prior_logprec, B, T, 1536, seg, W.pooled, 1536};
    run("xi_pool", 0, s, [&] { launch_xi_pool(a, s); });
    run("head", 0, s, [&] {
      launch_small_linear({W.pooled, 1536, head.wt, head.bias, embed, embed_dim, B, 1536, embed_dim, 0}, s);
    });
    return;
  }
  gemm("pool_linear1", pool1, xp, 1536, W.att, 128, M, T, 1, 0, kActTanh, s, seg, B, glob ? W.rowb : nullptr, !glob);
  if (opt.precision == 1 && opt.astp_fused) {
    AstpArgs a{W.att, xp, 1536, B, T, 1536, seg, pool2_frag, pool2.bias, 1e-7f, W.pooled};
    run("astp", 2.0 * M * 1536 * 128, s, [&] { launch_astp_fused(a, s); });
  } else {
    gemm("pool_linear2", pool2, W.att, 128, W.logit, 1536, M, T, 1, 0, kActNone, s, seg, B);
    run("astp", 0, s, [&] { launch_astp_pool(W.logit, xp, B, T, 1536, W.pooled, s, seg); });
  }
  run("head", 0, s, [&] {
    launch_small_linear({W.pooled, 3072, head.wt, head.bias, embed, embed_dim, B, 3072, embed_dim, 0}, s);
  });
}

}
```

wespeaker_hubert_amd/csrc/kernels.h:

```cpp
#pragma once

#include <vector>

#include "common.h"

namespace wsp {

enum AMode { kACat = 0, kAAdd = 1 };
enum Act { kActNone = 0, kActRelu = 1, kActTanh = 2, kActGelu = 3 };

struct ConvGemmArgs {
  const float* a[3];
  int lda[3];
  int cseg[4];
  int cin, taps, dil, pad;
  int M, T, N;
  const float* w;
  int K, Kp;
  const float* bias;
  const float* row_bias;
  const float* res;
  int ldres;
  const float* scale;
  const float* shift;
  float* out;
  int ldo;
  int act;
  int amode;
  int role;
  int conv2d;
  int Fi, Ti, Fo, To, stride, kw;
  int sc2d;
  int gcols, gcin;
  const int* seg;
  const int* iseg;
  int nseg;
  double* colsum;
  int lnmode;
  float* ln_out;
  const float* ln_in;
  int ln_parts;
  const float* ln_cs;
  const float* ln_g;
  const float* ln_b;
  float ln_eps;
  const float* gate;
  int ldg, gate_k0;
  const float* seam_h;
  int ld_seam_h;
  float* seam_out;
  int ld_seam_out;
};

inline ConvGemmArgs normalized(ConvGemmArgs p) {
  if (!p.conv2d && !p.sc2d) {
    if (p.stride <= 0) p.stride = 1;
    if (p.Ti <= 0) p.Ti = p.T;
  }
  return p;
}

int conv_gemm_x3_block_rows(const ConvGemmArgs& p, int variant);
void launch_colsum_mean(const double* part, int block_rows, int T, int B, int N, float* out, int ldo,
                        hipStream_t s);
void launch_conv_gemm_x3(const ConvGemmArgs& p, const void* whi, const void* wlo, int variant,
                         hipStream_t s);
bool conv_gemm_x3_gate_ok(const ConvGemmArgs& p, int variant);
bool conv_gemm_x3_seam_ok(const ConvGemmArgs& p, int variant);


void launch_conv_gemm(const ConvGemmArgs& p, hipStream_t s);
int conv_gemm_tile_for(int N);

struct SmallLinearArgs {
  const float* in;
  int ldin;
  const float* wt;
  const float* bias;
  float* out;
  int ldo;
  int R, K, N;
  int act;
  float* scratch = nullptr;
  size_t scratch_floats = 0;
};
void launch_small_linear(const SmallLinearArgs& p, hipStream_t s);
size_t small_linear_scratch_floats(int R, int N, int K);


void launch_frame_stats(const float* x, int ldx, int B, int T, int C, float* out, int ldo,
                        int with_std, int std_off, hipStream_t s, const int* seg = nullptr);

void launch_residual_scale(const float* x, const float* h, const float* g, float* out, int B,
                           int T, int C, hipStream_t s, const int* seg = nullptr, int M = 0);

void launch_astp_pool(const float* e, const float* x, int B, int T, int C, float* out,
                      hipStream_t s, const int* seg = nullptr, float var_floor = 1e-7f);

int simam_chunks(int B, int rows);
void launch_simam(const float* z, const float* res, float* out, int B, int rows, int C, double* part, float* coef,
                  hipStream_t s);
void launch_nhwc_to_tfc(const float* in, float* out, int B, int F, int T, int C, hipStream_t s);

void launch_resnet_stem(const float* feats, int B, int T, int F, int C0, const float* w, const float* bias,
                        float* out, hipStream_t s);

struct FbankConfig {
  int num_bins = 80, sample_rate = 16000, window = 0;
  double frame_length_ms = 25.0, frame_shift_ms = 10.0, low_freq = 20.0, high_freq = 0.0;
  int frame_len = 0, frame_shift = 0, padded = 0;
};
void fbank_config_resolve(FbankConfig& c);
void fbank_mel_banks(const FbankConfig& c, std::vector<float>& w);
struct FbankPlan {
  FbankConfig cfg;
  bool fixed = false;
  int len0 = 0, len1 = 0;
  std::vector<double> host_tab;
  const double* tab = nullptr;
};
void fbank_plan(const FbankConfig& c, FbankPlan& p);
void launch_fbank(const void* wav, int dtype, int B, int N, int ld, float scale, float* feats,
                  int T, int cmn, const FbankPlan& plan, hipStream_t s, const int* wseg = nullptr,
                  const int* fseg = nullptr);

void launch_hubert_conv0(const float* wav, int B, int N, int ldw, int T0, const float* w, const float* gamma,
                         const float* beta, double* stats, float* out, hipStream_t s, const int* wseg = nullptr,
                         const int* oseg = nullptr);
size_t hubert_conv0_stats_doubles(int B, int T0);
void launch_hubert_pos_conv(const float* x, int ldx, const int* seg, int B, int maxT, int M, const void* whi,
                            const void* wlo, int ldw, int gout, const float* bias, float* out, int ldo,
                            hipStream_t s);
struct LayerNormArgs {
  const float* x;
  int ldx;
  const float* add;
  int ldadd, gin, gout;
  const float* gamma;
  const float* beta;
  float eps;
  float* out;
  int ldo;
  int M, D;
  float* feat;
  float feat_w;
  int feat_init, T, Tout;
  const int* seg;
  const int* fseg;
  int nseg;
};
void launch_layernorm(const LayerNormArgs& p, hipStream_t s);
void launch_cmn_rows(float* x, int B, int T, int D, hipStream_t s, const int* seg = nullptr);
void launch_cmvn_rows(float* x, int B, int T, int D, int norm_mean, int norm_var, hipStream_t s,
                      const int* seg = nullptr);

void launch_l2_normalize(const float* x, const float* sub, float* y, int R, int D, hipStream_t s);
void launch_cosine_pairs(const float* E, int D, const int32_t* ia, const int32_t* ib, int P,
                         double* score, hipStream_t s);
void asnorm_layout(int Ne, int Nc, int D, int* Ncp, int* Dp, size_t* bytes);
void launch_asnorm_stats(const float* E, int Ne, const float* C, int Nc, int D, int top_n,
                         double* mu, double* sd, float* ws, hipStream_t s);
void launch_row_mean_accum(const float* x, const int32_t* group, int R, int D, double* acc,
                           double* cnt, hipStream_t s);

struct ResamplePlan {
  int orig = 1, nw = 1, width = 0, L = 1;
  bool identity = true;
  std::vector<float> kern;
  std::vector<int> band;
};
void resample_plan(int orig_freq, int new_freq, int lowpass_filter_width, double rolloff, ResamplePlan& p);
long long resample_out_len(const ResamplePlan& p, long long n);
void launch_resample(const ResamplePlan& p, const float* d_kern, const int* d_band, const float* x, int B, int N,
                     long ldx, float* y, long ldy, hipStream_t s);

}
```

wespeaker_hubert_amd/csrc/model.cpp:

```cpp
#include "model_impl.h"

namespace wsp {

int detail::chunk_for(int B, size_t bytes) {
  const int bc = std::min((int)std::max<size_t>(1, kOperandCap / bytes), B);
  const int chunks = (B + bc - 1) / bc;
  return (B + chunks - 1) / chunks;
}

void Model::Impl::add(const std::string& n, std::vector<int64_t> shape) {
  idx[n] = (int)params.size();
  params.push_back(Param{n, std::move(shape), {}, false});
}
void Model::Impl::add_bn(const std::string& p, int64_t c) {
  add(p + ".weight", {c});
  add(p + ".bias", {c});
  add(p + ".running_mean", {c});
  add(p + ".running_var", {c});
  add(p + ".num_batches_tracked", {});
}
const std::vector<float>& Model::Impl::P(const std::string& n) const {
  auto it = idx.find(n);
  WSP_CHECK(it != idx.end(), "missing parameter " + n);
  const Param& p = params[it->second];
  WSP_CHECK(p.set || p.numel() == 0, "parameter not set: " + n);
  return p.host;
}

void Model::Impl::bn_affine(const std::string& p, std::vector<double>& sc, std::vector<double>& sh) const {
  const auto& w = P(p + ".weight");
  const auto& b = P(p + ".bias");
  const auto& rm = P(p + ".running_mean");
  const auto& rv = P(p + ".running_var");
  sc.resize(w.size());
  sh.resize(w.size());
  for (size_t i = 0; i < w.size(); ++i) {
    sc[i] = (double)w[i] / std::sqrt((double)rv[i] + kBnEps);
    sh[i] = (double)b[i] - (double)rm[i] * sc[i];
  }
}

Model::Impl::Folded Model::Impl::fold_bn(const std::string& wname, const std::string& bn) const {
  std::vector<double> sc, sh;
  bn_affine(bn, sc, sh);
  Folded f{P(wname), std::vector<float>(sh.begin(), sh.end())};
  const size_t K = f.w.size() / sc.size();
  for (size_t i = 0; i < f.w.size(); ++i) f.w[i] = (float)(f.w[i] * sc[i / K]);
  return f;
}

ConvW Model::Impl::pack_conv(const std::vector<float>& w, int N, int cin, int taps, const float* bias,
                             const std::string& bn) {
  ConvW cw;
  cw.N = N;
  cw.cin = cin;
  cw.taps = taps;
  cw.K = cin * taps;
  cw.Kp = round_up(cw.K, 64);
  const std::vector<float> packed = pack::conv_kmajor(w, N, cin, taps, cw.Kp);
  std::vector<uint16_t> hi, lo;
  pack::split(packed, hi, lo);
  cw.w = dev.upload(packed);
  cw.whi = dev.upload_u16(hi);
  cw.wlo = dev.upload_u16(lo);
  if (bias) cw.bias = dev.upload(std::vector<float>(bias, bias + N));
  if (!bn.empty()) {
    std::vector<double> sc, sh;
    bn_affine(bn, sc, sh);
    cw.scale = dev.upload(std::vector<float>(sc.begin(), sc.end()));
    cw.shift = dev.upload(std::vector<float>(sh.begin(), sh.end()));
  }
  return cw;
}

LinW Model::Impl::pack_lin(const float* w, int N, int K, int ldk, const float* bias) {
  LinW lw;
  lw.N = N;
  lw.K = K;
  lw.wt = dev.upload(pack::transpose(w, N, K, ldk));
  if (bias) lw.bias = dev.upload(std::vector<float>(bias, bias + N));
  return lw;
}

void Model::Impl::one_operand(ConvGemmArgs& g, const float* a, int lda, int cin) {
  g.a[0] = g.a[1] = g.a[2] = a;
  g.lda[0] = g.lda[1] = g.lda[2] = lda;
  g.cseg[0] = 0;
  g.cseg[1] = g.cseg[2] = g.cseg[3] = cin;
}

void Model::Impl::fill(ConvGemmArgs& g, const ConvW& cw, int M, int T, int dil, int pad, float* out, int ldo, int act,
                       const float* row_bias, bool use_bias, const int* seg, int nseg) {
  g.cin = cw.cin;
  g.taps = cw.taps;
  g.dil = dil;
  g.pad = pad;
  g.M = M;
  g.T = T;
  g.N = cw.N;
  g.w = cw.w;
  g.K = cw.K;
  g.Kp = cw.Kp;
  g.bias = use_bias ? cw.bias : nullptr;
  g.row_bias = row_bias;
  g.scale = cw.scale;
  g.shift = cw.shift;
  g.out = out;
  g.ldo = ldo;
  g.act = act;
  g.seg = seg;
  g.nseg = nseg;
}

void Model::Impl::launch(const ConvGemmArgs& g, const ConvW& cw, hipStream_t s) {
  if (opt.precision == 1)
    launch_conv_gemm_x3(g, cw.whi, cw.wlo, opt.x3_variant, s);
  else
    launch_conv_gemm(g, s);
}

void Model::Impl::gemm(const char* tag, const ConvW& cw, const float* a0, int lda, float* out, int ldo, int M, int T,
                       int dil, int pad, int act, hipStream_t s, const int* seg, int nseg, const float* row_bias,
                       bool use_bias, int role) {
  ConvGemmArgs g{};
  one_operand(g, a0, lda, cw.cin);
  g.role = role;
  fill(g, cw, M, T, dil, pad, out, ldo, act, row_bias, use_bias, seg, nseg);
  run(tag, 2.0 * M * cw.N * cw.K, s, [&] { launch(g, cw, s); });
}

void Model::Impl::fork(hipStream_t s, int ns) {
  while ((int)sub_st.size() < ns - 1) {
    hipStream_t t;
    WSP_HIP(hipStreamCreateWithFlags(&t, hipStreamNonBlocking));
    sub_st.push_back(t);
  }
  while ((int)sub_ev.size() < ns) {
    hipEvent_t e;
    WSP_HIP(hipEventCreateWithFlags(&e, hipEventDisableTiming));
    sub_ev.push_back(e);
  }
  WSP_HIP(hipEventRecord(sub_ev[0], s));
  for (int i = 1; i < ns; ++i) WSP_HIP(hipStreamWaitEvent(sub_st[i - 1], sub_ev[0], 0));
}
void Model::Impl::join(hipStream_t s, int ns) {
  for (int i = 1; i < ns; ++i) {
    WSP_HIP(hipEventRecord(sub_ev[i], sub_st[i - 1]));
    WSP_HIP(hipStreamWaitEvent(s, sub_ev[i], 0));
  }
}

Model::Impl::~Impl() {
  for (auto& kv : prof_map)
    for (auto& e : kv.second.ev) {
      (void)hipEventDestroy(e.first);
      (void)hipEventDestroy(e.second);
    }
  for (auto t : sub_st) (void)hipStreamDestroy(t);
  for (auto e : sub_ev) (void)hipEventDestroy(e);
}

Model::~Model() { delete impl; }

void Model::create(const std::string& arch, int feat_dim, int embed_dim, bool emb_bn, bool two_emb) {
  WSP_CHECK(!impl, "model already created");
  for (MakeImpl* make : {make_ecapa, make_resnet, make_hubert, make_campplus, make_eres2net, make_gemini, make_xvec})
    if ((impl = make(arch, feat_dim, embed_dim, emb_bn, two_emb))) break;
  WSP_CHECK(impl, "unsupported arch " + arch);
  if (hipGetDevice(&impl->device) != hipSuccess) {
    (void)hipGetLastError();
    impl->device = -1;
  }
  impl->build_params();
}

int Model::num_params() const { return (int)impl->params.size(); }

void Model::param_info(int i, const char** name, int* ndim, int64_t* shape) const {
  WSP_CHECK(i >= 0 && i < num_params(), "param index out of range");
  const Param& p = impl->params[i];
  *name = p.name.c_str();
  *ndim = (int)p.shape.size();
  for (size_t d = 0; d < p.shape.size() && d < 4; ++d) shape[d] = p.shape[d];
}

void Model::set_param(int i, const float* data, int64_t numel) {
  WSP_CHECK(i >= 0 && i < num_params(), "param index out of range");
  Param& p = impl->params[i];
  WSP_CHECK(numel == p.numel(), "numel mismatch for " + p.name);
  p.host.assign(data, data + numel);
  p.set = true;
}

void Model::finalize() {
  Impl& m = *impl;
  WSP_CHECK(!m.finalized, "model already finalized");
  int dev = 0;
  WSP_HIP(hipGetDevice(&dev));
  WSP_CHECK(m.device < 0 || dev == m.device, "finalize on a different device than create");
  m.device = dev;
  for (auto& p : m.params)
    WSP_CHECK(p.set || p.name.find("num_batches_tracked") != std::string::npos,
              "parameter not set: " + p.name);
  m.finalize();
  for (auto& p : m.params) std::vector<float>().swap(p.host);
  m.finalized = true;
}

int Model::embed_dim() const { return impl->embed_dim; }
int Model::feat_dim() const { return impl->feat_dim; }

size_t Model::workspace_bytes(int B, int T) const {
  WSP_CHECK(!impl->is_frontend(), "HuBERT handle: use the front-end workspace query");
  const int ns = impl->nsub(B);
  size_t bytes = 256;
  for (int i = 0; i < ns; ++i) bytes += impl->ws_bytes_one(B * (i + 1) / ns - B * i / ns, T);
  return bytes;
}

void Model::forward(const float* feats, int B, int T, float* embed, void* ws, size_t ws_bytes,
                    hipStream_t s) {
  Impl& m = *impl;
  WSP_CHECK(!m.is_frontend(), "HuBERT handle: use the front-end forward");
  WSP_CHECK(m.finalized, "forward before finalize");
  if (m.min_frames() >= 2)
    WSP_CHECK(B > 0 && T > 1, "forward needs B >= 1 and T >= 2 frames");
  else
    WSP_CHECK(B > 0 && T >= 1, "forward needs B >= 1 and T >= 1 frames");
  WSP_CHECK((size_t)B * T < (1u << 31), "B*T too large");
  WSP_CHECK(ws_bytes >= workspace_bytes(B, T), "workspace too small");
  m.check_forward(B, T);
  char* wsb = reinterpret_cast<char*>((reinterpret_cast<uintptr_t>(ws) + 255) & ~uintptr_t(255));
  const int ns = m.nsub(B);
  if (ns > 1) m.fork(s, ns);
  for (int i = 0; i < ns; ++i) {
    const int b0 = B * i / ns, nb = B * (i + 1) / ns - b0;
    const float* f = feats + (size_t)b0 * T * m.feat_dim;
    float* e = embed + (size_t)b0 * m.embed_dim;
    m.forward(f, nb, T, e, reinterpret_cast<float*>(wsb), m.sub(s, i));
    wsb += m.ws_bytes_one(nb, T);
  }
  if (ns > 1) m.join(s, ns);
}

size_t Model::workspace_bytes_segments(int B, int M) const {
  WSP_CHECK(impl->has_segments(), "segmented batches are implemented for ECAPA-TDNN handles");
  WSP_CHECK(B > 0 && M >= B, "segmented batch needs B >= 1 and M >= B rows");
  return impl->ws_floats_segments(B, M) * sizeof(float) + 256;
}

void Model::forward_segments(const float* feats, int B, const int* seg, int M, float* embed, void* ws,
                             size_t ws_bytes, hipStream_t s) {
  Impl& m = *impl;
  WSP_CHECK(m.has_segments(), "segmented batches are implemented for ECAPA-TDNN handles");
  WSP_CHECK(m.finalized, "forward before finalize");
  WSP_CHECK(seg != nullptr && B > 0 && M >= B, "segmented batch needs offsets, B >= 1 and M >= B rows");
  WSP_CHECK((size_t)M * 1536 < (1u << 31) / 4, "segmented batch too large");
  WSP_CHECK(ws_bytes >= workspace_bytes_segments(B, M), "workspace too small");
  float* wsf = reinterpret_cast<float*>((reinterpret_cast<uintptr_t>(ws) + 255) & ~uintptr_t(255));
  m.forward_segments(feats, B, seg, M, embed, wsf, s);
}

void Model::profile(bool on) {
  if (on && !impl->prof)
    for (auto& kv : impl->prof_map) {
      kv.second.used = 0;
      kv.second.flops = 0;
    }
  impl->prof = on;
}

namespace {
struct Opt {
  const char* key;
  int Options::*field;
  int lo, hi, hole;
  const char* err;
};
using I = Options;
constexpr int kNoHole = -1000;
const Opt kOpts[] = {
    {"precision", &I::precision, 0, 1, kNoHole, "precision must be 0 (f32) or 1 (bf16x3)"},
    {"streams", &I::streams, 1, 8, kNoHole, "streams must be 1..8"},
    {"layer", &I::layer, -1, 12, kNoHole, "layer must be -1 (weighted sum) or 0..12"},
    {"in_planes", &I::in_planes, 32, 64, kNoHole, "in_planes must be 32 or 64"},
    {"res2_fused", &I::res2_fused, 0, 1, kNoHole, "res2_fused must be 0 or 1"},
    {"cam_fused", &I::cam_fused, 0, 1, kNoHole, "cam_fused must be 0 (separate BN-ReLU pass) or 1 (GEMM prologue)"},
    {"ib_fused", &I::ib_fused, 0, 1, kNoHole, "ib_fused must be 0 (conv1, depthwise conv, conv3) or 1 (conv1, fused tail)"},
    {"cat_gate", &I::cat_gate, 0, 1, kNoHole, "cat_gate must be 0 or 1"},
    {"gate_fold", &I::gate_fold, 0, 1, kNoHole, "gate_fold must be 0 or 1"},
    {"seam_fold", &I::seam_fold, 0, 1, kNoHole, "seam_fold must be 0 or 1"},
    {"res_prefetch", &I::res_prefetch, 0, 1, kNoHole, "res_prefetch must be 0 or 1"},
    {"res_tail", &I::res_tail, 0, 2, kNoHole, "res_tail must be 0 (off), 1 (tail + next conv1) or 2 (tail alone)"},
    {"sc_fuse", &I::sc_fuse, 0, 3, kNoHole, "sc_fuse must be 0 .. 3 (bit 0: one GEMM, bit 1: in the tail)"},
    {"c1_stage_fuse", &I::c1_stage_fuse, 0, 1, kNoHole, "c1_stage_fuse must be 0 or 1"},
    {"astp_fused", &I::astp_fused, 0, 3, kNoHole,
     "astp_fused must be 0 (linear2 GEMM + pooling kernel) or 1 (fused)"},
    {"attn_pipe", &I::attn_pipe, 0, 1, kNoHole, "attn_pipe must be 0 or 1"},
    {"pos_conv", &I::pos_conv, 0, 1, kNoHole,
     "pos_conv must be 0 (grouped implicit GEMM) or 1 (direct grouped conv)"},
    {"ln_fold", &I::ln_fold, 0, 1, kNoHole, "ln_fold must be 0 (LayerNorm kernels) or 1 (folded into the GEMMs)"},
    {"tail_batch", &I::tail_batch, 0, 1, kNoHole,
     "tail_batch must be 0 (CNN layers 4-6 per chunk) or 1 (batch-wide)"},
    {"res2_variant", &I::res2_variant, 0, 4, 1,
     "res2_variant must be 0 (4 waves, 2 x 2), 2 (4 waves on N, 4 W k-steps in flight), 3 (8 waves) "
     "or 4 (halo-free strips, c1024 widths; else as 3)"},
    {"x3_variant", &I::x3_variant, 0, 9, kNoHole,
     "x3_variant must be 3, 4, 5, 6 (5 on 16x16x32 MFMAs) or 7 (6 staged by LDS-DMA)"},
    {"conv3x3_img", &I::conv3x3_img, 0, 3, kNoHole,
     "conv3x3_img must be 0 (off), 1 (32 / 64 channels) or 2 / 3 (also 128)"},
};
const Opt& find_opt(const std::string& key) {
  for (const Opt& o : kOpts)
    if (key == o.key) return o;
  throw InvalidArg{"unknown option " + key};
}
}

void Model::set_option(const std::string& key, int value) {
  Impl& m = *impl;
  if (key == "attn_lds" || key == "conv1x1_rows") return;
  const Opt& o = find_opt(key);
  if (key == "layer") {
    WSP_CHECK(m.owns_option(key), "option 'layer' applies to the HuBERT front end");
    WSP_CHECK(!m.finalized, "option 'layer' must be set before finalize");
  } else if (key == "in_planes") {
    WSP_CHECK(m.owns_option(key), "option 'in_planes' applies to SimAM-ResNet handles");
    WSP_CHECK(!m.finalized, "option 'in_planes' must be set before finalize");
    WSP_CHECK(value == 32 || value == 64, o.err);
    for (const auto& p : m.params) WSP_CHECK(!p.set, "option 'in_planes' must be set before the weights");
  }
  WSP_CHECK(value >= o.lo && value <= o.hi && value != o.hole, o.err);
  if (key == "x3_variant") {
    value = value >= 3 && value <= 7 ? value : value == 8 ? 7 : 5;
  } else if (key == "astp_fused") {
    value = value ? 1 : 0;
  }
  m.opt.*o.field = value;
  if (key == "in_planes") m.build_params();
}

int Model::get_option(const std::string& key) const { return impl->opt.*find_opt(key).field; }

void Model::profile_query(const std::string& tag, int* launches, double* total_ms, double* flops) {
  *launches = 0;
  *total_ms = 0;
  *flops = 0;
  double fl = 0;
  for (auto& kv : impl->prof_map) {
    const std::string& k = kv.first;
    if (k != tag && k.compare(0, tag.size() + 1, tag + ".") != 0) continue;
    ProfEntry& e = kv.second;
    for (size_t i = 0; i < e.used; ++i) {
      WSP_HIP(hipEventSynchronize(e.ev[i].second));
      float ms = 0;
      WSP_HIP(hipEventElapsedTime(&ms, e.ev[i].first, e.ev[i].second));
      *total_ms += ms;
    }
    *launches += (int)e.used;
    fl += e.flops;
  }
  *flops = *launches ? fl / (double)*launches : 0.0;
}

}
```

wespeaker_hubert_amd/csrc/model_impl.h:

```cpp
#pragma once

#include <hip/hip_runtime.h>

#include <cmath>
#include <cstdint>
#include <algorithm>
#include <map>
#include <string>
#include <vector>

#include "kernels.h"
#include "model.h"
#include "pack.h"

namespace wsp {

namespace detail {

constexpr double kBnEps = 1e-5;

struct DevBuf {
  std::vector<void*> ptrs;
  ~DevBuf() {
    for (void* p : ptrs) (void)hipFree(p);
  }
  template <typename T>
  T* upload(const std::vector<T>& v) {
    void* p = nullptr;
    WSP_HIP(hipMalloc(&p, std::max<size_t>(v.size(), 1) * sizeof(T)));
    ptrs.push_back(p);
    if (!v.empty()) WSP_HIP(hipMemcpy(p, v.data(), v.size() * sizeof(T), hipMemcpyHostToDevice));
    return static_cast<T*>(p);
  }
  void* upload_u16(const std::vector<uint16_t>& v) { return upload(v); }
};

struct ConvW {
  float* w = nullptr;
  void* whi = nullptr;
  void* wlo = nullptr;
  float* bias = nullptr;
  float* scale = nullptr;
  float* shift = nullptr;
  int N = 0, cin = 0, taps = 1, K = 0, Kp = 0;
  void* frag = nullptr;
};

struct LinW {
  float* wt = nullptr;
  float* bias = nullptr;
  int K = 0, N = 0;
};

inline int round_up(int a, int b) { return (a + b - 1) / b * b; }

constexpr size_t kOperandCap = ((size_t)1 << 31) / 8 * 7;
int chunk_for(int B, size_t bytes);

struct WsCursor {
  float* base = nullptr;
  size_t off = 0;
  static size_t padded(size_t n) { return (n + 63) / 64 * 64; }
  float* take(size_t n) {
    float* p = base ? base + off : nullptr;
    off += padded(n);
    return p;
  }
};

}

using namespace detail;

struct Param {
  std::string name;
  std::vector<int64_t> shape;
  std::vector<float> host;
  bool set = false;
  int64_t numel() const {
    int64_t n = 1;
    for (auto s : shape) n *= s;
    return n;
  }
};

struct ProfEntry {
  std::vector<std::pair<hipEvent_t, hipEvent_t>> ev;
  size_t used = 0;
  double flops = 0;
};

struct Options {
  int precision = 1;
  int x3_variant = 5;
  int streams = 1;
  int res2_fused = 1;
  int res2_variant = 4;
  int cat_gate = 1;
  int gate_fold = 1;
  int seam_fold = 1;
  int astp_fused = 1;
  int in_planes = 32;
  int conv3x3_img = 2;
  int res_prefetch = 1;
  int res_tail = 1;
  int sc_fuse = 3;
  int c1_stage_fuse = 1;
  int layer = -1;
  int attn_pipe = 1;
  int pos_conv = 1;
  int ln_fold = 0;
  int tail_batch = 1;
  int cam_fused = 1;
  int ib_fused = 0;
};

struct Model::Impl {
  std::string arch;
  int feat_dim = 80, embed_dim = 192;
  bool emb_bn = false, two_emb = false;
  Options opt;
  std::vector<Param> params;
  std::map<std::string, int> idx;
  bool finalized = false;
  int device = 0;
  DevBuf dev;

  Impl(const std::string& arch, int feat_dim, int embed_dim, bool emb_bn, bool two_emb)
      : arch(arch), feat_dim(feat_dim), embed_dim(embed_dim), emb_bn(emb_bn), two_emb(two_emb) {}
  virtual ~Impl();

  virtual void build_params() = 0;
  virtual void finalize() = 0;
  virtual bool owns_option(const std::string&) const { return false; }
  virtual bool is_frontend() const { return false; }
  virtual void check_forward(int B, int T) const {}
  virtual int min_frames() const { return 2; }
  virtual size_t ws_floats(int B, int T) const = 0;
  virtual void forward(const float* feats, int B, int T, float* embed, float* ws, hipStream_t s) = 0;
  virtual bool has_segments() const { return false; }
  virtual size_t ws_floats_segments(int B, int M) const { return 0; }
  virtual void forward_segments(const float* feats, int B, const int* seg, int M, float* embed, float* ws,
                                hipStream_t s) {}

  std::vector<hipStream_t> sub_st;
  std::vector<hipEvent_t> sub_ev;
  int nsub(int B) const { return std::max(1, std::min(opt.streams, B)); }
  size_t ws_bytes_one(int B, int T) const { return (ws_floats(B, T) * sizeof(float) + 255) & ~size_t(255); }
  hipStream_t sub(hipStream_t s, int i) const { return i == 0 ? s : sub_st[i - 1]; }
  void fork(hipStream_t s, int ns);
  void join(hipStream_t s, int ns);

  void add(const std::string& n, std::vector<int64_t> shape);
  void add_bn(const std::string& p, int64_t c);
  const std::vector<float>& P(const std::string& n) const;
  void bn_affine(const std::string& p, std::vector<double>& sc, std::vector<double>& sh) const;
  struct Folded {
    std::vector<float> w, b;
  };
  Folded fold_bn(const std::string& wname, const std::string& bn) const;

  ConvW pack_conv(const std::vector<float>& w, int N, int cin, int taps, const float* bias, const std::string& bn);
  void* pack_frag(const std::vector<float>& w, int N, int K, pack::FragOrder order = pack::kPlain, int kacc = -1) {
    return dev.upload_u16(pack::frag(w, N, K, order, kacc));
  }
  void* pack_frag_acc(const std::vector<float>& w, int N, int K, int kacc = -1) { return pack_frag(w, N, K, pack::kAcc, kacc); }
  LinW pack_lin(const float* w, int N, int K, int ldk, const float* bias);

  static void one_operand(ConvGemmArgs& g, const float* a, int lda, int cin);
  void fill(ConvGemmArgs& g, const ConvW& cw, int M, int T, int dil, int pad, float* out, int ldo, int act,
            const float* row_bias, bool use_bias, const int* seg, int nseg);
  void launch(const ConvGemmArgs& g, const ConvW& cw, hipStream_t s);
  void gemm(const char* tag, const ConvW& cw, const float* a0, int lda, float* out, int ldo, int M, int T, int dil,
            int pad, int act, hipStream_t s, const int* seg, int nseg, const float* row_bias = nullptr,
            bool use_bias = true, int role = 0);

  bool prof = false;
  std::map<std::string, ProfEntry> prof_map;
  template <typename F>
  void run(const char* tag, double flops, hipStream_t s, F&& f) {
    if (!prof) {
      f();
      return;
    }
    ProfEntry& e = prof_map[tag];
    if (e.used == e.ev.size()) {
      hipEvent_t a, b;
      WSP_HIP(hipEventCreate(&a));
      WSP_HIP(hipEventCreate(&b));
      e.ev.emplace_back(a, b);
    }
    auto& pr = e.ev[e.used++];
    e.flops += flops;
    WSP_HIP(hipEventRecord(pr.first, s));
    f();
    WSP_HIP(hipEventRecord(pr.second, s));
  }
};

using MakeImpl = Model::Impl*(const std::string& arch, int feat_dim, int embed_dim, bool emb_bn, bool two_emb);
MakeImpl make_ecapa, make_resnet, make_hubert, make_campplus, make_eres2net, make_gemini, make_xvec;

}
```

wespeaker_hubert_amd/csrc/res2_chain.h:

```cpp
#pragma once

#include "common.h"

namespace wsp {

struct Res2Args {
  const float* x;
  float* out;
  int ldx, ldo, M, T, dil, rout;
  const int* seg;
  int nseg;
  const void* w;
  const float* bias;
  const float* scale;
  const float* shift;
  int variant;
};
bool res2_chain_supported(int w, int dil);
int res2_chain_rout(int dil, int variant, int M);
void launch_res2_chain(const Res2Args& p, int w, hipStream_t s);

}
```

wespeaker_hubert_amd/csrc/res2_chain.hip:

```cpp
#include <algorithm>
#include <type_traits>

#include "bf16x3.h"
#include "gemm_common.h"
#include "res2_chain.h"

namespace wsp {

namespace {

constexpr int kPad = 4;

template <int W, int R, int WNv, int NWv = R / 32>
struct Geo {
  static constexpr int IR = R + 2 * kPad;
  static constexpr int RB = 2 * W;
  static constexpr int PLANE = (IR + 1) * RB;
  static constexpr int KS = 3 * W / 16;
  static constexpr int KC = W / 16;
  static constexpr int WST = 64 * W;
  static constexpr int NW = NWv;
  static constexpr int WN = WNv, WM = NW / WN, TM = R / 32 / WM, TN = W / 32 / WN;
  static_assert(TN >= 1 && TM >= 1, "res2 wave layout");
  static constexpr int NT = NW * 64;
  static constexpr int LDS = 2 * PLANE;
  __device__ __forceinline__ static int sw(int ir) { return W == 128 ? (ir & 15) : ((ir >> 1) & 7); }
  __device__ __forceinline__ static int addr(int ir, int ch) {
    return ir * RB + (((ch >> 3) ^ sw(ir)) << 4) + (ch & 7) * 2;
  }
};

__device__ __forceinline__ unsigned short bf_bits(__bf16 x) { return __builtin_bit_cast(unsigned short, x); }

template <int W, int R, int WNv, int NWv, int PD>
__global__ __launch_bounds__(NWv * 64, R == 128 ? NWv / 2 : 1) void res2_chain_kernel(const Res2Args p) {
  using G = Geo<W, R, WNv, NWv>;
  constexpr int TM = G::TM, TN = G::TN, NT = G::NT, IR = G::IR;
  extern __shared__ __attribute__((aligned(16))) unsigned char smem[];
  unsigned char* xhi = smem;
  unsigned char* xlo = smem + G::PLANE;

  const int tid = threadIdx.x;
  const int lane = tid & 63;
  const int wave = tid >> 6;
  const int wm = wave / G::WN;
  const int wn = wave - wm * G::WN;
  const int r32 = lane & 31;
  const int h = lane >> 5;
  const int d = p.dil;
  const int blk = xcd_remap(blockIdx.x, gridDim.x);
  const int own0 = blk * p.rout;
  const int own1 = min(own0 + p.rout, p.M);
  const int wr0 = own0 - 6 * d;

  if (tid < G::RB / 4) {
    reinterpret_cast<unsigned*>(xhi + IR * G::RB)[tid] = 0u;
    reinterpret_cast<unsigned*>(xlo + IR * G::RB)[tid] = 0u;
  }
  const __amdgpu_buffer_rsrc_t rx = make_rsrc(p.x);
  constexpr int C4 = W / 4;
  for (int q = tid; q < IR * C4; q += NT) {
    const int ir = q / C4;
    const int c = (q - ir * C4) * 4;
    const int m = wr0 + ir - kPad;
    const f32x4 v = bload4(rx, (m >= 0 && m < p.M) ? (m * p.ldx + c) * 4 : kOOB);
    bf16x4 hi, lo;
    split(v, hi, lo);
    const int a = G::addr(ir, c);
    *reinterpret_cast<bf16x4*>(xhi + a) = hi;
    *reinterpret_cast<bf16x4*>(xlo + a) = lo;
  }

  int arow[TM][3], asw[TM][3];
#pragma unroll
  for (int i = 0; i < TM; ++i) {
    const int r = (wm * TM + i) * 32 + r32;
    const int m = wr0 + r;
    int t = -1, L = 0;
    if (m >= 0 && m < p.M) {
      if (p.seg) {
        const int u = seg_of(p.seg, p.nseg, m);
        t = m - p.seg[u];
        L = p.seg[u + 1] - p.seg[u];
      } else {
        const int u = m / p.T;
        t = m - u * p.T;
        L = p.T;
      }
    }
#pragma unroll
    for (int j = 0; j < 3; ++j) {
      const int off = (j - 1) * d;
      const bool ok = t >= 0 && t + off >= 0 && t + off < L;
      const int ir = ok ? r + off + kPad : IR;
      arow[i][j] = ir * G::RB;
      asw[i][j] = G::sw(ir);
    }
  }

  constexpr int kTotal = 7 * G::KS;
  const __amdgpu_buffer_rsrc_t rw = make_rsrc(p.w);
  const int wlane = (wn * TN * 64 + lane) * 16;
  auto wload = [&](int g, bf16x8 (&bh)[TN], bf16x8 (&bl)[TN]) {
    const bool ok = g < kTotal;
#pragma unroll
    for (int j = 0; j < TN; ++j) {
      const int o = (g * 2 * (W / 32) + j) * 1024 + wlane;
      bh[j] = __builtin_bit_cast(bf16x8, __builtin_amdgcn_raw_buffer_load_b128(rw, ok ? o : kOOB, 0, 0));
      bl[j] = __builtin_bit_cast(bf16x8, __builtin_amdgcn_raw_buffer_load_b128(rw, ok ? o + (W / 32) * 1024 : kOOB, 0, 0));
    }
  };
  static_assert(PD % 2 == 0 && G::KS % PD == 0, "res2 W prefetch depth");
  bf16x8 wbh[PD][TN], wbl[PD][TN];
#pragma unroll
  for (int d = 0; d < PD; ++d) wload(d, wbh[d], wbl[d]);
  __syncthreads();

  const __amdgpu_buffer_rsrc_t rout = make_rsrc(p.out);
  f32x16 acc[TM][TN];
  auto read_a = [&](int t, bf16x8 (&ah)[TM], bf16x8 (&al)[TM]) {
    const int tap = t / G::KC, q = (t % G::KC) * 2 + h;
#pragma unroll
    for (int i = 0; i < TM; ++i) {
      const int ar = tap == 0 ? arow[i][0] : tap == 1 ? arow[i][1] : arow[i][2];
      const int as = tap == 0 ? asw[i][0] : tap == 1 ? asw[i][1] : asw[i][2];
      const int a = ar + ((q ^ as) << 4);
      ah[i] = *reinterpret_cast<const bf16x8*>(xhi + a);
      al[i] = *reinterpret_cast<const bf16x8*>(xlo + a);
    }
  };
  auto mma = [&](int g, const bf16x8 (&ah)[TM], const bf16x8 (&al)[TM], bf16x8 (&bh)[TN], bf16x8 (&bl)[TN]) {
#pragma unroll
    for (int i = 0; i < TM; ++i)
#pragma unroll
      for (int j = 0; j < TN; ++j) mma3(ah[i], al[i], bh[j], bl[j], acc[i][j]);
    wload(g + PD, bh, bl);
  };
  bf16x8 ah2[2][TM], al2[2][TM];

#pragma unroll 1
  for (int step = 0; step < 7; ++step) {
    const int gb = step * G::KS;
#pragma unroll
    for (int i = 0; i < TM; ++i)
#pragma unroll
      for (int j = 0; j < TN; ++j)
#pragma unroll
        for (int r = 0; r < 16; ++r) acc[i][j][r] = 0.f;
    read_a(0, ah2[0], al2[0]);
#pragma unroll 1
    for (int t = 0; t < G::KS - PD; t += PD) {
#pragma unroll
      for (int u = 0; u < PD; ++u) {
        read_a(t + u + 1, ah2[(u + 1) & 1], al2[(u + 1) & 1]);
        mma(gb + t + u, ah2[u & 1], al2[u & 1], wbh[u], wbl[u]);
      }
    }
    int ldx4 = p.ldx * 4, ldo4 = p.ldo * 4, mw = wr0 + wm * TM * 32 + 4 * h;
    asm volatile("" : "+s"(ldx4), "+s"(ldo4), "+v"(mw));
    float nx[TM][TN][16];
    if (step < 6) {
      const __amdgpu_buffer_rsrc_t rxs = make_rsrc(p.x);
#pragma unroll
      for (int i = 0; i < TM; ++i) {
        const int m0 = mw + i * 32;
        const int lo = -m0, hi = p.M - m0;
#pragma unroll
        for (int j = 0; j < TN; ++j) {
          const int base = (m0 * p.ldx + (step + 1) * W + (wn * TN + j) * 32 + r32) * 4;
#pragma unroll
          for (int r = 0; r < 16; ++r) {
            const int rr = (r & 3) + 8 * (r >> 2);
            nx[i][j][r] = __builtin_bit_cast(
                float, __builtin_amdgcn_raw_buffer_load_b32(rxs, (rr >= lo && rr < hi) ? base + rr * ldx4 : kOOB, 0, 0));
          }
        }
      }
    }
#pragma unroll
    for (int u = 0; u < PD; ++u) {
      if (u + 1 < PD) read_a(G::KS - PD + u + 1, ah2[(u + 1) & 1], al2[(u + 1) & 1]);
      mma(gb + G::KS - PD + u, ah2[u & 1], al2[u & 1], wbh[u], wbl[u]);
    }
    __syncthreads();

#pragma unroll
    for (int j = 0; j < TN; ++j) {
      const int col = (wn * TN + j) * 32 + r32;
      const float bv = p.bias[step * W + col];
      const float sc = p.scale[step * W + col];
      const float sh = p.shift[step * W + col];
#pragma unroll
      for (int i = 0; i < TM; ++i) {
        const int m0 = mw + i * 32;
        const int olo = own0 - m0, ohi = own1 - m0;
        const int base = (m0 * p.ldo + step * W + col) * 4;
        const int irb = m0 - wr0 + kPad;
#pragma unroll
        for (int r = 0; r < 16; ++r) {
          const int rr = (r & 3) + 8 * (r >> 2);
          const float y = fmaxf(acc[i][j][r] + bv, 0.f) * sc + sh;
          __builtin_amdgcn_raw_buffer_store_b32(__builtin_bit_cast(unsigned, y), rout,
                                                (rr >= olo && rr < ohi) ? base + rr * ldo4 : kOOB, 0, 0);
          if (step < 6) {
            const float x = y + nx[i][j][r];
            const __bf16 hh = (__bf16)x;
            const __bf16 ll = (__bf16)(x - (float)hh);
            const unsigned send = (lane & 1) ? bf_bits(hh) : bf_bits(ll);
            const unsigned recv = (unsigned)__builtin_amdgcn_mov_dpp((int)send, 0xB1, 0xF, 0xF, false);
            const int a = G::addr(irb + rr, col & ~1);
            if (lane & 1)
              *reinterpret_cast<unsigned*>(xlo + a) = recv | ((unsigned)bf_bits(ll) << 16);
            else
              *reinterpret_cast<unsigned*>(xhi + a) = (unsigned)bf_bits(hh) | (recv << 16);
          }
        }
      }
    }
    __syncthreads();
  }
}

constexpr int kSR = 96;
constexpr int kSIR = kSR + 2 * kPad;
constexpr int kSRB = 256;
constexpr int kSPlane = (kSIR + 1) * kSRB + 64;
constexpr int kSHistRows = 2 * kPad;
constexpr int kSLds = 2 * kSPlane + 6 * kSHistRows * 2 * kSRB;
static_assert(kSR % 16 == 0, "history rows keep their swizzle only if kSR % 16 == 0");
static_assert(2 * kSLds <= 160 * 1024, "two strip blocks per CU");

__device__ __forceinline__ int s_off(int ir, int ch) { return ((((ch >> 3) ^ (ir & 15)) << 4)) + (ch & 7) * 2; }

template <int PD>
__global__ __launch_bounds__(256, 2) void res2_strip_kernel(const Res2Args p) {
  constexpr int W = 128, KS = 3 * W / 16, KC = W / 16, TM = 3, kTotal = 7 * KS;
  static_assert(KS % PD == 0 && PD % 2 == 0, "res2 strip W prefetch depth");
  extern __shared__ __attribute__((aligned(16))) unsigned char smem[];
  unsigned char* xhi = smem;
  unsigned char* xlo = smem + kSPlane;
  unsigned char* hist = smem + 2 * kSPlane;

  const int tid = threadIdx.x;
  const int lane = tid & 63;
  const int wn = tid >> 6;
  const int r32 = lane & 31;
  const int h = lane >> 5;
  const int d = p.dil;
  const int M = p.M;
  const int blk = xcd_remap(blockIdx.x, gridDim.x);
  const int own0 = blk * p.rout;
  const int own1 = min(own0 + p.rout, M);
  const int r0 = own0 - 6 * d;
  const int nch = (own1 - own0 + 12 * d + kSR - 1) / kSR;

  if (tid < kSRB / 4) {
    reinterpret_cast<unsigned*>(xhi + kSIR * kSRB)[tid] = 0u;
    reinterpret_cast<unsigned*>(xlo + kSIR * kSRB)[tid] = 0u;
  }
  for (int q = tid; q < 6 * kSHistRows * 2 * kSRB / 16; q += 256)
    reinterpret_cast<u32x4*>(hist)[q] = u32x4{0u, 0u, 0u, 0u};
  const __amdgpu_buffer_rsrc_t rx = make_rsrc(p.x);
  auto put4 = [&](int ir, int c, const f32x4& v) {
    bf16x4 hi, lo;
    split(v, hi, lo);
    const int a = ir * kSRB + s_off(ir, c);
    *reinterpret_cast<bf16x4*>(xhi + a) = hi;
    *reinterpret_cast<bf16x4*>(xlo + a) = lo;
  };
  for (int q = tid; q < (kSR + 2 * d) * (W / 4); q += 256) {
    const int ir = q / (W / 4);
    const int c = (q - ir * (W / 4)) * 4;
    const int m = r0 - d + ir;
    put4(ir, c, bload4(rx, (m >= 0 && m < M) ? (m * p.ldx + c) * 4 : kOOB));
  }

  const __amdgpu_buffer_rsrc_t rw = make_rsrc(p.w);
  const int wlane = (wn * 64 + lane) * 16;
  auto wload = [&](int g, bf16x8& bh, bf16x8& bl) {
    const int o = g * 2 * (W / 32) * 1024 + wlane;
    bh = __builtin_bit_cast(bf16x8, __builtin_amdgcn_raw_buffer_load_b128(rw, o, 0, 0));
    bl = __builtin_bit_cast(bf16x8, __builtin_amdgcn_raw_buffer_load_b128(rw, o + (W / 32) * 1024, 0, 0));
  };
  bf16x8 wbh[PD], wbl[PD];
#pragma unroll
  for (int u = 0; u < PD; ++u) wload(u, wbh[u], wbl[u]);
  __syncthreads();

  const __amdgpu_buffer_rsrc_t rout = make_rsrc(p.out);
  const __amdgpu_buffer_rsrc_t rbias = make_rsrc(p.bias);
  const __amdgpu_buffer_rsrc_t rscale = make_rsrc(p.scale);
  const __amdgpu_buffer_rsrc_t rshift = make_rsrc(p.shift);
  f32x16 acc[TM];
  int vm[TM];
  int dq = d;
  auto read_a = [&](auto na, int t, bf16x8 (&ah)[TM], bf16x8 (&al)[TM]) {
    constexpr int NA = decltype(na)::value;
    const int tap = t / KC, q = (t % KC) * 2 + h;
#pragma unroll
    for (int i = 0; i < NA; ++i) {
      const int ir = ((vm[i] >> tap) & 1) ? i * 32 + r32 + tap * dq : kSIR;
      const int a = ir * kSRB + ((q ^ (ir & 15)) << 4);
      ah[i] = *reinterpret_cast<const bf16x8*>(xhi + a);
      al[i] = *reinterpret_cast<const bf16x8*>(xlo + a);
    }
    __builtin_amdgcn_sched_barrier(0);
  };
  auto mma = [&](auto na, int g, const bf16x8 (&ah)[TM], const bf16x8 (&al)[TM], bf16x8& bh, bf16x8& bl) {
    constexpr int NA = decltype(na)::value;
#pragma unroll
    for (int i = 0; i < NA; ++i) mma3(ah[i], al[i], bh, bl, acc[i]);
    const int gn = g + PD;
    wload(gn >= kTotal ? gn - kTotal : gn, bh, bl);
    __builtin_amdgcn_sched_barrier(0);
  };
  bf16x8 ah2[2][TM], al2[2][TM];
  const int col = wn * 32 + r32;

  auto conv_step = [&](auto na, int c, int step, bool more) {
    constexpr int NA = decltype(na)::value;
        const int base = r0 + c * kSR - step * d;
        dq = d;
        asm volatile("" : "+s"(dq));
  #pragma unroll
        for (int i = 0; i < NA; ++i) {
          const int lr = i * 32 + r32;
          const int m = base + lr;
          int t = -1, L = 0;
          if (m >= 0 && m < M) {
            if (p.seg) {
              const int u = seg_of(p.seg, p.nseg, m);
              t = m - p.seg[u];
              L = p.seg[u + 1] - p.seg[u];
            } else {
              const int u = m / p.T;
              t = m - u * p.T;
              L = p.T;
            }
          }
          int v = 0;
  #pragma unroll
          for (int j = 0; j < 3; ++j) {
            const int tt = t + (j - 1) * d;
            v |= (t >= 0 && tt >= 0 && tt < L) ? 1 << j : 0;
          }
          vm[i] = v;
        }
  #pragma unroll
        for (int i = 0; i < NA; ++i)
  #pragma unroll
          for (int r = 0; r < 16; ++r) acc[i][r] = 0.f;
        const int gb = step * KS;
        const float bv = __builtin_bit_cast(float, __builtin_amdgcn_raw_buffer_load_b32(rbias, (step * W + col) * 4, 0, 0));
        const float sc = __builtin_bit_cast(float, __builtin_amdgcn_raw_buffer_load_b32(rscale, (step * W + col) * 4, 0, 0));
        const float sh = __builtin_bit_cast(float, __builtin_amdgcn_raw_buffer_load_b32(rshift, (step * W + col) * 4, 0, 0));
        read_a(na, 0, ah2[0], al2[0]);
  #pragma unroll 1
        for (int t = 0; t < KS - PD; t += PD) {
  #pragma unroll
          for (int u = 0; u < PD; ++u) {
            read_a(na, t + u + 1, ah2[(u + 1) & 1], al2[(u + 1) & 1]);
            mma(na, gb + t + u, ah2[u & 1], al2[u & 1], wbh[u], wbl[u]);
          }
        }
        const bool wimg = step < 6 || more;
        int ldx4 = p.ldx * 4, ldo4 = p.ldo * 4;
        int abase = step < 6 ? base : r0 + (c + 1) * kSR + d;
        asm volatile("" : "+s"(ldx4), "+s"(ldo4), "+s"(abase));
        const int acol = step < 6 ? (step + 1) * W : 0;
        float nx[TM][16];
        f32x4 xh = {0.f, 0.f, 0.f, 0.f};
        if (wimg) {
  #pragma unroll
          for (int i = 0; i < NA; ++i) {
            const int m0 = abase + i * 32 + 4 * h;
            const int lo = -m0, hi = M - m0;
            const int b0 = (m0 * p.ldx + acol + col) * 4;
            if (abase + i * 32 >= 0 && abase + i * 32 + 32 <= M) {
  #pragma unroll
              for (int r = 0; r < 16; ++r)
                nx[i][r] = __builtin_bit_cast(
                    float, __builtin_amdgcn_raw_buffer_load_b32(rx, b0, ((r & 3) + 8 * (r >> 2)) * ldx4, 0));
            } else {
  #pragma unroll
              for (int r = 0; r < 16; ++r) {
                const int rr = (r & 3) + 8 * (r >> 2);
                nx[i][r] = __builtin_bit_cast(
                    float, __builtin_amdgcn_raw_buffer_load_b32(rx, (rr >= lo && rr < hi) ? b0 + rr * ldx4 : kOOB, 0, 0));
              }
            }
          }
          if (step == 6 && tid < 2 * d * (W / 4)) {
            const int k = tid / (W / 4), c4 = (tid - k * (W / 4)) * 4;
            const int m = r0 + (c + 1) * kSR - d + k;
            xh = bload4(rx, (m >= 0 && m < M) ? (m * p.ldx + c4) * 4 : kOOB);
          }
        }
  #pragma unroll
        for (int u = 0; u < PD; ++u) {
          if (u + 1 < PD) read_a(na, KS - PD + u + 1, ah2[(u + 1) & 1], al2[(u + 1) & 1]);
          mma(na, gb + KS - PD + u, ah2[u & 1], al2[u & 1], wbh[u], wbl[u]);
        }
        __syncthreads();

        const int cp = col & ~1;
        unsigned char* hslot = hist + (step - 1) * (kSHistRows * 2 * kSRB);
        const bool odd = lane & 1;
        const int ib = 2 * dq + 4 * h;
        int a4[4];
#pragma unroll
        for (int k = 0; k < 4; ++k) a4[k] = (ib + k) * kSRB + s_off(ib + k, cp);
        unsigned char* img = xhi + (odd ? kSPlane : 0);
        auto epi = [&](auto mode_, auto full_) {
          constexpr int MODE = decltype(mode_)::value;
          constexpr bool FULL = decltype(full_)::value;
#pragma unroll
          for (int i = 0; i < NA; ++i) {
            const int lr0 = i * 32 + 4 * h;
            const int m0 = base + lr0;
            const int olo = own0 - m0, ohi = own1 - m0;
            const int b0 = (m0 * p.ldo + step * W + col) * 4;
#pragma unroll
            for (int r = 0; r < 16; ++r) {
              const int rr = (r & 3) + 8 * (r >> 2);
              const float y = fmaxf(acc[i][r] + bv, 0.f) * sc + sh;
              if constexpr (FULL)
                __builtin_amdgcn_raw_buffer_store_b32(__builtin_bit_cast(unsigned, y), rout, b0, rr * ldo4, 0);
              else
                __builtin_amdgcn_raw_buffer_store_b32(__builtin_bit_cast(unsigned, y), rout,
                                                      rr >= olo && rr < ohi ? b0 + rr * ldo4 : kOOB, 0, 0);
              if constexpr (MODE != 0) {
                const float x = MODE == 1 ? y + nx[i][r] : nx[i][r];
                const __bf16 hh = (__bf16)x;
                const __bf16 ll = (__bf16)(x - (float)hh);
                const unsigned send = odd ? bf_bits(hh) : bf_bits(ll);
                const unsigned recv = (unsigned)__builtin_amdgcn_mov_dpp((int)send, 0xB1, 0xF, 0xF, false);
                const int ir = ib + 32 * i + rr;
                const int a = ((r >> 2) & 1 ? (a4[r & 3] ^ 128) + 8 * kSRB : a4[r & 3]) + ((r >> 3) * 16 + 32 * i) * kSRB;
                unsigned* dst = reinterpret_cast<unsigned*>(img + a);
                if (NA == TM && i == TM - 1 && ir >= kSR) {
                  if (step >= 1)
                    *reinterpret_cast<unsigned*>(hslot + ((ir - kSR) * 2 + (lane & 1)) * kSRB + (a - ir * kSRB)) = *dst;
                }
                *dst = odd ? (recv | ((unsigned)bf_bits(ll) << 16)) : ((unsigned)bf_bits(hh) | (recv << 16));
              }
            }
          }
        };
        const bool full = base >= own0 && base + NA * 32 <= own1;
        if (!wimg) epi(std::integral_constant<int, 0>{}, std::false_type{});
        else if (step == 6) epi(std::integral_constant<int, 2>{}, std::false_type{});
        else if (full) epi(std::integral_constant<int, 1>{}, std::true_type{});
        else epi(std::integral_constant<int, 1>{}, std::false_type{});
        if (step < 6) {
          if (tid < 2 * d * 32) {
            const int k = tid >> 5, pl = (tid >> 4) & 1, e = tid & 15;
            const u32x4 v = reinterpret_cast<const u32x4*>(hist + step * (kSHistRows * 2 * kSRB) + (k * 2 + pl) * kSRB)[e];
            reinterpret_cast<u32x4*>((pl ? xlo : xhi) + k * kSRB)[e] = v;
          }
        } else if (more && tid < 2 * d * (W / 4)) {
          const int k = tid / (W / 4), c4 = (tid - k * (W / 4)) * 4;
          put4(k, c4, xh);
        }
  };

  const int last_tiles = (own1 - own0 + 12 * d - (nch - 1) * kSR + 31) / 32;
#pragma unroll 1
  for (int c = 0; c < nch; ++c) {
    const bool more = c + 1 < nch;
    const int nt = more ? TM : last_tiles;
#pragma unroll 1
    for (int step = 0; step < 7; ++step) {
      if (nt >= 3) conv_step(std::integral_constant<int, 3>{}, c, step, more);
      else if (nt == 2) conv_step(std::integral_constant<int, 2>{}, c, step, more);
      else conv_step(std::integral_constant<int, 1>{}, c, step, more);
      __syncthreads();
    }
  }
}

}

bool res2_chain_supported(int w, int dil) { return (w == 64 || w == 128) && dil >= 1 && dil <= kPad; }

static int res2_rows(int) { return 128; }

template <int W, int R, int WN, int NW = R / 32, int PD = 2>
void launch_res2_k(const Res2Args& p, int nblk, hipStream_t s) {
  hipLaunchKernelGGL((res2_chain_kernel<W, R, WN, NW, PD>), dim3(nblk), dim3(Geo<W, R, WN, NW>::NT),
                     (Geo<W, R, WN, NW>::LDS), s, p);
}

template <int W>
void launch_res2_w(const Res2Args& p, int nblk, hipStream_t s) {
  if (W == 128 && p.variant == 4) {
    hipLaunchKernelGGL(res2_strip_kernel<4>, dim3(nblk), dim3(256), kSLds, s, p);
  } else if (p.variant == 3) {
    if constexpr (W == 128) launch_res2_k<W, 128, 4, 8>(p, nblk, s);
    else launch_res2_k<W, 128, 2, 8>(p, nblk, s);
  } else if (p.variant == 2) {
    if constexpr (W == 128) launch_res2_k<W, 128, 4, 4, 4>(p, nblk, s);
    else launch_res2_k<W, 128, 2>(p, nblk, s);
  } else {
    launch_res2_k<W, 128, 2>(p, nblk, s);
  }
}

void launch_res2_chain(const Res2Args& p, int w, hipStream_t s) {
  WSP_CHECK(res2_chain_supported(w, p.dil), "res2_chain: width must be 64 or 128 and dilation 1..4");
  WSP_CHECK(p.M > 0 && (p.seg || p.T > 0), "res2_chain: empty shape");
  WSP_CHECK(p.rout == res2_chain_rout(p.dil, p.variant, p.M), "res2_chain: rout must be res2_chain_rout(dil, variant, M)");
  WSP_CHECK((long long)p.M * p.ldx * 4 < (long long)kOOB && (long long)p.M * p.ldo * 4 < (long long)kOOB,
            "res2_chain: operand exceeds 2 GiB (split the batch)");
  WSP_CHECK(p.ldx >= 8 * w && p.ldo >= 7 * w && p.ldx % 4 == 0, "res2_chain: bad leading dimensions");
  const int nblk = (p.M + p.rout - 1) / p.rout;
  if (w == 128)
    launch_res2_w<128>(p, nblk, s);
  else
    launch_res2_w<64>(p, nblk, s);
  WSP_HIP(hipGetLastError());
}

int res2_chain_rout(int dil, int variant, int M) {
  if (variant == 4) return std::max(64, ceil_div(M, 2 * device_cu_count()));
  return res2_rows(variant) - 12 * dil;
}

}
```

Baseline: 25910.

## Store producer outputs pre-split into packed bf16 hi/lo words for conv3 A operands

Adds a packed (x3p) activation format. The res2 strip kernel, the conv1 epilogue for its tail columns, and the seam output now write each fp32 value as interleaved bf16 hi/lo pairs. The consuming conv3 and conv_cat GEMMs then read those K ranges straight as bf16 fragments and skip the per-tile fp32-to-bf16x3 split in the inner loop. This moves split work out of the hot MFMA loop into producer epilogues. In exchange it adds more template variants, DPP lane swaps in the epilogues, and coupling between kernels through the new layout, enabled by default behind an a_packed option.

```diff
diff --git a/wespeaker_hubert_amd/csrc/conv_gemm.hip b/wespeaker_hubert_amd/csrc/conv_gemm.hip
--- a/wespeaker_hubert_amd/csrc/conv_gemm.hip
+++ b/wespeaker_hubert_amd/csrc/conv_gemm.hip
@@ -135,8 +135,10 @@
   WSP_CHECK(!p.colsum, "conv_gemm: column sums are a bf16x3-kernel epilogue");
   WSP_CHECK(!p.conv2d && p.N % 64 == 0, "conv_gemm (f32): 1-D convs with N % 64 == 0 only");
   WSP_CHECK(!p.gcols || p.gcols % 64 == 0, "conv_gemm (f32): grouped columns must be a multiple of 64");
-  WSP_CHECK(!p.sc2d && !p.lnmode && !p.gate && !p.seam_h && !p.seam_out,
-            "conv_gemm (f32): conv3 + shortcut, the LayerNorm fold, the gated A tail and the seam run on tile family 7");
+  WSP_CHECK(!p.sc2d && !p.lnmode && !p.gate && !p.seam_h && !p.seam_out && !p.pk_k0 && !p.pk_k1 && !p.out_pk_from &&
+                !p.seam_out_pk,
+            "conv_gemm (f32): conv3 + shortcut, the LayerNorm fold, the gated A tail, the seam and packed (x3p) "
+            "operands run on tile family 7");
   if (conv_gemm_tile_for(p.N) == 0 && !p.gcols)
     launch_tile<2, 2, 2, 2>(p, s);
   else
diff --git a/wespeaker_hubert_amd/csrc/conv_gemm_x3.hip b/wespeaker_hubert_amd/csrc/conv_gemm_x3.hip
--- a/wespeaker_hubert_amd/csrc/conv_gemm_x3.hip
+++ b/wespeaker_hubert_amd/csrc/conv_gemm_x3.hip
@@ -40,10 +40,18 @@
   return variant == 7 && args.seam_h && x3::seam_supported(normalized(args));
 }
 
+static bool has_packed(const ConvGemmArgs& p) { return p.pk_k0 || p.pk_k1 || p.out_pk_from || p.seam_out_pk; }
+
+bool conv_gemm_x3_packed_ok(const ConvGemmArgs& args, int variant) {
+  return variant == 7 && has_packed(args) && x3::g256_packed_supported(normalized(args));
+}
+
 void launch_conv_gemm_x3(const ConvGemmArgs& args, const void* whi, const void* wlo, int variant,
                          hipStream_t s) {
   const ConvGemmArgs p = normalized(args);
   check_conv_args(p, "conv_gemm_x3");
+  WSP_CHECK(!has_packed(p) || (variant == 7 && x3::g256_packed_supported(p)),
+            "conv_gemm_x3: packed (x3p) operands run on tile family 7 only (conv_gemm_x3_packed_ok)");
   if (p.colsum) {
     const int bm = conv_gemm_x3_block_rows(p, variant);
     WSP_CHECK(!p.seg && !p.row_bias && !p.conv2d && p.T >= bm,
diff --git a/wespeaker_hubert_amd/csrc/conv_gemm_x3_g.h b/wespeaker_hubert_amd/csrc/conv_gemm_x3_g.h
--- a/wespeaker_hubert_amd/csrc/conv_gemm_x3_g.h
+++ b/wespeaker_hubert_amd/csrc/conv_gemm_x3_g.h
@@ -17,6 +17,25 @@
 constexpr int kGEpiLd = 132;
 constexpr int kGEpiBytes = 8 * 32 * kGEpiLd * 4;
 typedef unsigned u32x4 __attribute__((ext_vector_type(4)));
+typedef unsigned u32x2 __attribute__((ext_vector_type(2)));
+
+__device__ __forceinline__ u32x4 g_x3p_words(u32x2 h, u32x2 l, int lane) {
+  const bool odd = lane & 1;
+  auto swap = [](unsigned v) { return (unsigned)__builtin_amdgcn_mov_dpp((int)v, 0xB1, 0xF, 0xF, false); };
+  const unsigned r0 = swap(odd ? h[0] : l[0]), r1 = swap(odd ? h[1] : l[1]);
+  return odd ? u32x4{r0, r1, l[0], l[1]} : u32x4{h[0], h[1], r0, r1};
+}
+__device__ __forceinline__ u32x4 g_x3p_pair(const f32x4& v, int lane) {
+#pragma clang fp contract(off)
+  bf16x4 hi, lo;
+#pragma unroll
+  for (int e = 0; e < 4; ++e) {
+    const __bf16 hh = (__bf16)v[e];
+    hi[e] = hh;
+    lo[e] = (__bf16)(v[e] - (float)hh);
+  }
+  return g_x3p_words(__builtin_bit_cast(u32x2, hi), __builtin_bit_cast(u32x2, lo), lane);
+}
 
 constexpr int kLnMaxParts = 8;
 __device__ __forceinline__ void g_ln_row(const ConvGemmArgs& p, int row, float& mu, float& rstd) {
@@ -83,6 +102,8 @@
   const int lparts = p.N / 128, lpart = (n0 + wn * 128) / 128;
   const __amdgpu_buffer_rsrc_t ro = make_rsrc(p.out);
   const __amdgpu_buffer_rsrc_t rres = make_rsrc(RES ? p.res : p.out);
+  bool pko = false;
+  if constexpr (!RB && !RES && LNM == 0) pko = p.out_pk_from > 0 && n0 + wn * 128 >= p.out_pk_from;
 #pragma unroll
   for (int h = 0; h < 2; ++h) {
     float pm[(LNM & 1) ? 16 : 1], pm2[(LNM & 1) ? 16 : 1];
@@ -128,8 +149,11 @@
         else if constexpr (ACT == kActGelu) v = gelu_as(v);
         y[e] = v * sc[e] + sh[e];
       }
-      __builtin_amdgcn_raw_buffer_store_b128(__builtin_bit_cast(u32x4, y), ro, ok ? (row * p.ldo + col) * 4 : kOOB, 0,
-                                             0);
+      u32x4 yst = __builtin_bit_cast(u32x4, y);
+      if constexpr (!RB && !RES && LNM == 0) {
+        if (pko) yst = g_x3p_pair(y, lane);
+      }
+      __builtin_amdgcn_raw_buffer_store_b128(yst, ro, ok ? (row * p.ldo + col) * 4 : kOOB, 0, 0);
       if constexpr ((LNM & 1) != 0) {
         pm[u] = ((y[0] + y[1]) + (y[2] + y[3])) * 0.25f;
         float q2 = 0.f;
diff --git a/wespeaker_hubert_amd/csrc/conv_gemm_x3_impl.h b/wespeaker_hubert_amd/csrc/conv_gemm_x3_impl.h
--- a/wespeaker_hubert_amd/csrc/conv_gemm_x3_impl.h
+++ b/wespeaker_hubert_amd/csrc/conv_gemm_x3_impl.h
@@ -326,6 +326,7 @@
 void t_4x2_2x4_mf16(const ConvGemmArgs&, const __bf16*, const __bf16*, hipStream_t);
 bool g256_supported(const ConvGemmArgs&);
 bool g256_gate_supported(const ConvGemmArgs&);
+bool g256_packed_supported(const ConvGemmArgs&);
 void t_g256(const ConvGemmArgs&, const __bf16*, const __bf16*, hipStream_t);
 bool seam_supported(const ConvGemmArgs&);
 void t_seam(const ConvGemmArgs&, const __bf16*, const __bf16*, hipStream_t, bool balanced = true);
diff --git a/wespeaker_hubert_amd/csrc/conv_gemm_x3_t6.hip b/wespeaker_hubert_amd/csrc/conv_gemm_x3_t6.hip
--- a/wespeaker_hubert_amd/csrc/conv_gemm_x3_t6.hip
+++ b/wespeaker_hubert_amd/csrc/conv_gemm_x3_t6.hip
@@ -93,7 +93,9 @@
   }
 }
 
-template <int AM, bool CSK, int LNM = 0>
+constexpr int kTF = 0, kTG = 1, kTP = 2;
+
+template <int AM, bool CSK, int LNM = 0, bool PK = false>
 __global__ __launch_bounds__(512, 1) void conv_gemm_g(const ConvGemmArgs p, const __bf16* __restrict__ whi,
                                                       const __bf16* __restrict__ wlo) {
   using L = Lds<true, 16>;
@@ -207,14 +209,19 @@
   bf16x8 ah[2], al[2], bh[4], bl[4];
   const int g_nb = GATE ? min((m0 / p.T + 1) * p.T, p.M) - m0 : 0;
   const int g_slot = GATE ? (p.K - p.gate_k0) * 4 : 0;
-  auto rdA = [&](auto gated, const unsigned char* st, int ih, const unsigned char* gp = nullptr) {
+  auto rdA = [&](auto kind, const unsigned char* st, int ih, const unsigned char* gp = nullptr) {
 #pragma clang fp contract(off)
 #pragma unroll
     for (int i = 0; i < 2; ++i) {
       const int r = wm * 64 + (ih * 2 + i) * 16 + r16;
+      if constexpr (decltype(kind)::value == kTP) {
+        ah[i] = *reinterpret_cast<const bf16x8*>(st + g_aslot(r, 2 * qk));
+        al[i] = *reinterpret_cast<const bf16x8*>(st + g_aslot(r, 2 * qk + 1));
+        continue;
+      }
       f32x4 x0 = *reinterpret_cast<const f32x4*>(st + g_aslot(r, 2 * qk));
       f32x4 x1 = *reinterpret_cast<const f32x4*>(st + g_aslot(r, 2 * qk + 1));
-      if constexpr (decltype(gated)::value) {
+      if constexpr (decltype(kind)::value == kTG) {
         const unsigned char* gr = gp + (r >= g_nb ? g_slot : 0);
         x0 = x0 * *reinterpret_cast<const f32x4*>(gr);
         x1 = x1 * *reinterpret_cast<const f32x4*>(gr + 16);
@@ -271,7 +278,7 @@
     const int buf = kt & 1;
     const unsigned char* st = smem + buf * kGStage;
     const unsigned char* gp =
-        decltype(gated)::value ? smem + 2 * kGStage + (kt * BK - p.gate_k0 + 8 * qk) * 4 : nullptr;
+        decltype(gated)::value == kTG ? smem + 2 * kGStage + (kt * BK - p.gate_k0 + 8 * qk) * 4 : nullptr;
     rdA(gated, st, 0, gp);
     rdB(st, 0);
     mm(0, 0);
@@ -286,10 +293,20 @@
     __builtin_amdgcn_sched_barrier(0);
     if (kt + 2 < nk) dma(kt + 2, buf);
   };
+  using TF = std::integral_constant<int, kTF>;
+  using TG = std::integral_constant<int, kTG>;
+  using TP = std::integral_constant<int, kTP>;
   const int ktg = GATE ? p.gate_k0 / BK : nk;
-  for (int kt = 0; kt < ktg; ++kt) ktile(std::false_type{}, kt);
+  const int kp0 = PK ? p.pk_k0 / BK : ktg, kp1 = PK ? p.pk_k1 / BK : ktg;
+  int kt = 0;
+  for (; kt < kp0; ++kt) ktile(TF{}, kt);
+  if constexpr (PK) {
+    for (; kt < kp1; ++kt) ktile(TP{}, kt);
+    if constexpr (!GATE)
+      for (; kt < ktg; ++kt) ktile(TF{}, kt);
+  }
   if constexpr (GATE)
-    for (int kt = ktg; kt < nk; ++kt) ktile(std::true_type{}, kt);
+    for (; kt < nk; ++kt) ktile(TG{}, kt);
 #define WSP_GEPI(RB, RES)                                                                                   \
   switch (p.act) {                                                                                         \
     case kActRelu: g_epilogue_rows<kActRelu, RB, RES>(p, acc, m0, n0, wm, wn, wave, lane, smem); break;    \
@@ -344,6 +361,27 @@
          (long long)(p.M / p.T) * p.ldg * 4 < (long long)kOOB;
 }
 
+bool g256_packed_supported(const ConvGemmArgs& p) {
+  if (!g256_supported(p) || !uniform_ktiles(p)) return false;
+  auto a16 = [](const void* q) { return (reinterpret_cast<uintptr_t>(q) & 15) == 0; };
+  if (p.pk_k0 || p.pk_k1) {
+    const bool dense = p.taps == 1 && p.pad == 0 && p.stride == 1 && !p.iseg && (p.seg || p.Ti == p.T);
+    auto edge = [&](int k) { return k == 0 || k == p.cseg[1] || k == p.cseg[2] || k == p.cin; };
+    const bool range = p.pk_k0 >= 0 && p.pk_k0 < p.pk_k1 && p.pk_k1 <= p.K && p.pk_k0 % 32 == 0 &&
+                       p.pk_k1 % 32 == 0 && edge(p.pk_k0) && edge(p.pk_k1);
+    const bool inst = p.gate ? g256_gate_supported(p) && p.pk_k1 == p.gate_k0 : p.colsum != nullptr;
+    if (!dense || !range || !inst || p.K != p.Kp || p.sc2d || p.lnmode || p.seam_h || !a16(p.a[0]) ||
+        !a16(p.a[1]) || !a16(p.a[2]))
+      return false;
+  }
+  if (p.out_pk_from) {
+    const bool plain = !p.res && !p.row_bias && !p.colsum && !p.lnmode && !p.sc2d;
+    if (!plain || p.out_pk_from < 0 || p.out_pk_from >= p.N || p.out_pk_from % 128 != 0) return false;
+  }
+  if (p.seam_out_pk && !(p.seam_h && seam_supported(p))) return false;
+  return true;
+}
+
 void t_g256(const ConvGemmArgs& p, const __bf16* h, const __bf16* l, hipStream_t s) {
   const int nwg = ((p.M + 255) / 256) * (p.N / 256);
   constexpr int lds0 = 2 * kGStage > kGEpiBytes ? 2 * kGStage : kGEpiBytes;
@@ -353,7 +391,15 @@
   if (p.gate) {
     WSP_CHECK(g256_gate_supported(p), "conv_gemm_x3: the gated A tail needs a dense 1x1 GEMM over a uniform batch");
     const int ldsg = std::max(lds, 2 * kGStage + 2 * (p.K - p.gate_k0) * 4);
-    hipLaunchKernelGGL((conv_gemm_g<4, false>), dim3(nwg), dim3(512), ldsg, s, p, h, l);
+    if (p.pk_k1)
+      hipLaunchKernelGGL((conv_gemm_g<4, false, 0, true>), dim3(nwg), dim3(512), ldsg, s, p, h, l);
+    else
+      hipLaunchKernelGGL((conv_gemm_g<4, false>), dim3(nwg), dim3(512), ldsg, s, p, h, l);
+    WSP_HIP(hipGetLastError());
+    return;
+  }
+  if (p.pk_k1) {
+    hipLaunchKernelGGL((conv_gemm_g<1, true, 0, true>), dim3(nwg), dim3(512), lds, s, p, h, l);
     WSP_HIP(hipGetLastError());
     return;
   }
diff --git a/wespeaker_hubert_amd/csrc/conv_gemm_x3_t7.hip b/wespeaker_hubert_amd/csrc/conv_gemm_x3_t7.hip
--- a/wespeaker_hubert_amd/csrc/conv_gemm_x3_t7.hip
+++ b/wespeaker_hubert_amd/csrc/conv_gemm_x3_t7.hip
@@ -6,7 +6,7 @@
 constexpr int kSPlane = 256 * 64;
 constexpr int kSStage = 4 * kSPlane;
 
-template <bool BAL>
+template <bool BAL, bool SPK = false>
 __global__ __launch_bounds__(512, 1) void conv_gemm_seam(const ConvGemmArgs p, const __bf16* __restrict__ whi,
                                                          const __bf16* __restrict__ wlo) {
   using L = Lds<true, 16>;
@@ -97,8 +97,10 @@
         hi[e] = hh;
         lo[e] = (__bf16)(v[e] - (float)hh);
       }
-      __builtin_amdgcn_raw_buffer_store_b128(__builtin_bit_cast(u32x4, v), rs,
-                                             mine && a_r[i] >= 0 ? (a_r[i] * p.ld_seam_out + kc) * 4 : kOOB, 0, 0);
+      u32x4 vst = __builtin_bit_cast(u32x4, v);
+      if constexpr (SPK) vst = g_x3p_words(__builtin_bit_cast(u32x2, hi), __builtin_bit_cast(u32x2, lo), tid);
+      __builtin_amdgcn_raw_buffer_store_b128(vst, rs, mine && a_r[i] >= 0 ? (a_r[i] * p.ld_seam_out + kc) * 4 : kOOB, 0,
+                                             0);
       const int off = L::off(srow + 64 * i, c8 * 8);
       *reinterpret_cast<bf16x4*>(st + off) = hi;
       *reinterpret_cast<bf16x4*>(st + kSPlane + off) = lo;
@@ -217,8 +219,12 @@
   WSP_CHECK(seam_supported(p), "conv_gemm_x3: the seam needs a dense 1x1 GEMM over a uniform batch with T >= 256");
   const int nwg = ((p.M + 255) / 256) * (p.N / 256);
   const int lds = std::max(2 * kSStage + 2 * p.K * 4, kGEpiBytes);
-  if (balanced)
+  if (balanced && p.seam_out_pk)
+    hipLaunchKernelGGL((conv_gemm_seam<true, true>), dim3(nwg), dim3(512), lds, s, p, h, l);
+  else if (balanced)
     hipLaunchKernelGGL((conv_gemm_seam<true>), dim3(nwg), dim3(512), lds, s, p, h, l);
+  else if (p.seam_out_pk)
+    hipLaunchKernelGGL((conv_gemm_seam<false, true>), dim3(nwg), dim3(512), lds, s, p, h, l);
   else
     hipLaunchKernelGGL((conv_gemm_seam<false>), dim3(nwg), dim3(512), lds, s, p, h, l);
   WSP_HIP(hipGetLastError());
diff --git a/wespeaker_hubert_amd/csrc/ecapa_model.cpp b/wespeaker_hubert_amd/csrc/ecapa_model.cpp
--- a/wespeaker_hubert_amd/csrc/ecapa_model.cpp
+++ b/wespeaker_hubert_amd/csrc/ecapa_model.cpp
@@ -276,20 +276,79 @@
     if (fold) gcat = g;
   }
 
+  auto c1_args = [&](int li) {
+    ConvGemmArgs g{};
+    one_operand(g, x[li + 1], C, C);
+    g.role = 1;
+    fill(g, blk[li].c1, M, T, 1, 0, h1, C, kActRelu, nullptr, true, seg, B);
+    return g;
+  };
+  auto seam_args = [&](int li) {
+    ConvGemmArgs g = c1_args(li);
+    fill(g, blk[li + 1].c1, M, T, 1, 0, h1, C, kActRelu, nullptr, true, seg, B);
+    g.seam_h = h3;
+    g.ld_seam_h = C;
+    g.gate = W.gate;
+    g.ldg = C;
+    g.seam_out = x[li + 2];
+    g.ld_seam_out = C;
+    return g;
+  };
+  auto c3_args = [&](int li) {
+    ConvGemmArgs g{};
+    g.amode = kACat;
+    g.a[0] = h2;
+    g.a[1] = h1 + 7 * w;
+    g.a[2] = h1;
+    g.cseg[1] = 7 * w;
+    g.cseg[2] = g.cseg[3] = C;
+    g.role = 1;
+    if (se_fused) g.colsum = W.sesum;
+    g.lda[0] = g.lda[1] = g.lda[2] = C;
+    fill(g, blk[li].c3, M, T, 1, 0, h3, C, kActRelu, nullptr, true, seg, B);
+    return g;
+  };
+  bool seamf[2];
+  for (int li = 0; li < 2; ++li)
+    seamf[li] = opt.seam_fold && opt.precision == 1 && conv_gemm_x3_seam_ok(seam_args(li), opt.x3_variant);
+  bool pk3 = false, pkx = false;
+  if (opt.a_packed && opt.precision == 1 && opt.res2_fused && w == 128 && opt.res2_variant == 4) {
+    pk3 = true;
+    for (int li = 0; li < 3; ++li) {
+      ConvGemmArgs g3 = c3_args(li);
+      g3.pk_k1 = C;
+      ConvGemmArgs g1 = li > 0 && seamf[li - 1] ? seam_args(li - 1) : c1_args(li);
+      g1.out_pk_from = 7 * w;
+      pk3 = pk3 && blk[li].r2w && conv_gemm_x3_packed_ok(g3, opt.x3_variant) &&
+            conv_gemm_x3_packed_ok(g1, opt.x3_variant);
+    }
+    if (pk3 && fold && seamf[1]) {
+      ConvGemmArgs gc = gcat, gs = seam_args(1);
+      gc.pk_k0 = C;
+      gc.pk_k1 = 2 * C;
+      gs.out_pk_from = 7 * w;
+      gs.seam_out_pk = 1;
+      pkx = conv_gemm_x3_packed_ok(gc, opt.x3_variant) && conv_gemm_x3_packed_ok(gs, opt.x3_variant);
+      if (pkx) gcat = gc;
+    }
+  }
+
   gemm("layer1", layer1, feats, feat_dim, x[1], C, M, T, 1, 2, kActRelu, s, seg, B);
-  ConvGemmArgs gseam{};
-  bool seam = false;
   for (int li = 0; li < 3; ++li) {
     const Block& b = blk[li];
     const int dil = li + 2;
     const float* xin = x[li + 1];
-    if (seam) {
+    if (li > 0 && seamf[li - 1]) {
+      ConvGemmArgs g = seam_args(li - 1);
+      g.out_pk_from = pk3 ? 7 * w : 0;
+      g.seam_out_pk = pkx && li == 2;
       run("se.scale", 0, s, [&] {
-        run("seam", 0, s, [&] { run("conv1x1_CxC", 2.0 * M * C * C, s, [&] { launch(gseam, b.c1, s); }); });
+        run("seam", 0, s, [&] { run("conv1x1_CxC", 2.0 * M * C * C, s, [&] { launch(g, b.c1, s); }); });
       });
-      seam = false;
     } else {
-      gemm("conv1x1_CxC", b.c1, xin, C, h1, C, M, T, 1, 0, kActRelu, s, seg, B, nullptr, true, 1);
+      ConvGemmArgs g = c1_args(li);
+      g.out_pk_from = pk3 ? 7 * w : 0;
+      run("conv1x1_CxC", 2.0 * M * C * C, s, [&] { launch(g, b.c1, s); });
     }
     if (opt.precision == 1 && opt.res2_fused && b.r2w) {
       Res2Args r{};
@@ -307,6 +366,7 @@
       r.bias = b.r2b;
       r.scale = b.r2s;
       r.shift = b.r2t;
+      r.out_pk = pk3;
       run("res2_k3", 7 * 2.0 * M * w * 3 * w, s, [&] { launch_res2_chain(r, w, s); });
     } else {
       for (int i = 0; i < 7; ++i) {
@@ -323,16 +383,11 @@
       }
     }
     {
-      ConvGemmArgs g{};
-      g.amode = kACat;
-      g.a[0] = h2;
-      g.a[1] = h1 + 7 * w;
-      g.a[2] = h1;
-      g.cseg[1] = 7 * w;
-      g.cseg[2] = g.cseg[3] = C;
-      g.role = 1;
-      if (se_fused) g.colsum = W.sesum;
-      gemm3("conv1x1_CxC", g, b.c3, 1, 0, h3, C);
+      ConvGemmArgs g = c3_args(li);
+      g.pk_k1 = pk3 ? C : 0;
+      auto c3 = [&] { run("conv1x1_CxC", 2.0 * M * C * C, s, [&] { launch(g, b.c3, s); }); };
+      if (pk3) run("packed", 0, s, c3);
+      else c3();
     }
     run("se", 0, s, [&] {
       if (se_fused) launch_colsum_mean(W.sesum, se_bm, T, B, C, W.gmean, C, s);
@@ -341,28 +396,13 @@
       launch_small_linear({W.ghid, 128, b.se2.wt, b.se2.bias, W.gate, C, B, 128, C, 3}, s);
     });
     if (li == 2 && fold) continue;
-    if (li < 2 && opt.seam_fold && opt.precision == 1) {
-      ConvGemmArgs g{};
-      one_operand(g, xin, C, C);
-      g.role = 1;
-      g.seam_h = h3;
-      g.ld_seam_h = C;
-      g.gate = W.gate;
-      g.ldg = C;
-      g.seam_out = x[li + 2];
-      g.ld_seam_out = C;
-      fill(g, blk[li + 1].c1, M, T, 1, 0, h1, C, kActRelu, nullptr, true, seg, B);
-      seam = conv_gemm_x3_seam_ok(g, opt.x3_variant);
-      if (seam) {
-        gseam = g;
-        continue;
-      }
-    }
+    if (li < 2 && seamf[li]) continue;
     run("se.scale", 0, s, [&] {
       launch_residual_scale(opt.cat_gate && li == 2 ? nullptr : xin, h3, W.gate, x[li + 2], B, T, C, s, seg, M);
     });
   }
-  gemm3("conv_cat", gcat, wcat, 1, 0, xp, 1536);
+  if (pkx) run("packed", 0, s, [&] { gemm3("conv_cat", gcat, wcat, 1, 0, xp, 1536); });
+  else gemm3("conv_cat", gcat, wcat, 1, 0, xp, 1536);
   if (glob) {
     run("glob_ctx", 0, s, [&] {
       launch_frame_stats(xp, 1536, B, T, 1536, W.gstats, 3072, 1, 1536, s, seg);
diff --git a/wespeaker_hubert_amd/csrc/kernels.h b/wespeaker_hubert_amd/csrc/kernels.h
--- a/wespeaker_hubert_amd/csrc/kernels.h
+++ b/wespeaker_hubert_amd/csrc/kernels.h
@@ -50,6 +50,9 @@
   int ld_seam_h;
   float* seam_out;
   int ld_seam_out;
+  int pk_k0, pk_k1;
+  int out_pk_from;
+  int seam_out_pk;
 };
 
 inline ConvGemmArgs normalized(ConvGemmArgs p) {
@@ -67,6 +70,7 @@
                          hipStream_t s);
 bool conv_gemm_x3_gate_ok(const ConvGemmArgs& p, int variant);
 bool conv_gemm_x3_seam_ok(const ConvGemmArgs& p, int variant);
+bool conv_gemm_x3_packed_ok(const ConvGemmArgs& p, int variant);
 
 
 void launch_conv_gemm(const ConvGemmArgs& p, hipStream_t s);
diff --git a/wespeaker_hubert_amd/csrc/model.cpp b/wespeaker_hubert_amd/csrc/model.cpp
--- a/wespeaker_hubert_amd/csrc/model.cpp
+++ b/wespeaker_hubert_amd/csrc/model.cpp
@@ -290,6 +290,7 @@
     {"cat_gate", &I::cat_gate, 0, 1, kNoHole, "cat_gate must be 0 or 1"},
     {"gate_fold", &I::gate_fold, 0, 1, kNoHole, "gate_fold must be 0 or 1"},
     {"seam_fold", &I::seam_fold, 0, 1, kNoHole, "seam_fold must be 0 or 1"},
+    {"a_packed", &I::a_packed, 0, 1, kNoHole, "a_packed must be 0 or 1"},
     {"res_prefetch", &I::res_prefetch, 0, 1, kNoHole, "res_prefetch must be 0 or 1"},
     {"res_tail", &I::res_tail, 0, 2, kNoHole, "res_tail must be 0 (off), 1 (tail + next conv1) or 2 (tail alone)"},
     {"sc_fuse", &I::sc_fuse, 0, 3, kNoHole, "sc_fuse must be 0 .. 3 (bit 0: one GEMM, bit 1: in the tail)"},
diff --git a/wespeaker_hubert_amd/csrc/model_impl.h b/wespeaker_hubert_amd/csrc/model_impl.h
--- a/wespeaker_hubert_amd/csrc/model_impl.h
+++ b/wespeaker_hubert_amd/csrc/model_impl.h
@@ -99,6 +99,7 @@
   int cat_gate = 1;
   int gate_fold = 1;
   int seam_fold = 1;
+  int a_packed = 1;
   int astp_fused = 1;
   int in_planes = 32;
   int conv3x3_img = 2;
diff --git a/wespeaker_hubert_amd/csrc/res2_chain.h b/wespeaker_hubert_amd/csrc/res2_chain.h
--- a/wespeaker_hubert_amd/csrc/res2_chain.h
+++ b/wespeaker_hubert_amd/csrc/res2_chain.h
@@ -15,6 +15,7 @@
   const float* scale;
   const float* shift;
   int variant;
+  int out_pk;
 };
 bool res2_chain_supported(int w, int dil);
 int res2_chain_rout(int dil, int variant, int M);
diff --git a/wespeaker_hubert_amd/csrc/res2_chain.hip b/wespeaker_hubert_amd/csrc/res2_chain.hip
--- a/wespeaker_hubert_amd/csrc/res2_chain.hip
+++ b/wespeaker_hubert_amd/csrc/res2_chain.hip
@@ -31,6 +31,8 @@
 };
 
 __device__ __forceinline__ unsigned short bf_bits(__bf16 x) { return __builtin_bit_cast(unsigned short, x); }
+typedef float f32x2 __attribute__((ext_vector_type(2)));
+typedef __bf16 bf16x2 __attribute__((ext_vector_type(2)));
 
 template <int W, int R, int WNv, int NWv, int PD>
 __global__ __launch_bounds__(NWv * 64, R == 128 ? NWv / 2 : 1) void res2_chain_kernel(const Res2Args p) {
@@ -232,7 +234,7 @@
 
 __device__ __forceinline__ int s_off(int ir, int ch) { return ((((ch >> 3) ^ (ir & 15)) << 4)) + (ch & 7) * 2; }
 
-template <int PD>
+template <int PD, bool PKO = false>
 __global__ __launch_bounds__(256, 2) void res2_strip_kernel(const Res2Args p) {
   constexpr int W = 128, KS = 3 * W / 16, KC = W / 16, TM = 3, kTotal = 7 * KS;
   static_assert(KS % PD == 0 && PD % 2 == 0, "res2 strip W prefetch depth");
@@ -411,6 +413,7 @@
 #pragma unroll
         for (int k = 0; k < 4; ++k) a4[k] = (ib + k) * kSRB + s_off(ib + k, cp);
         unsigned char* img = xhi + (odd ? kSPlane : 0);
+        const unsigned pk_sel0 = odd ? 0x01000504u : 0x05040100u, pk_sel1 = odd ? 0x03020706u : 0x07060302u;
         auto epi = [&](auto mode_, auto full_) {
           constexpr int MODE = decltype(mode_)::value;
           constexpr bool FULL = decltype(full_)::value;
@@ -419,16 +422,37 @@
             const int lr0 = i * 32 + 4 * h;
             const int m0 = base + lr0;
             const int olo = own0 - m0, ohi = own1 - m0;
-            const int b0 = (m0 * p.ldo + step * W + col) * 4;
+            const int b0 = PKO ? (m0 * p.ldo + step * W) * 4 + 32 * (cp >> 3) + 2 * (cp & 7) + (odd ? 16 : 0)
+                               : (m0 * p.ldo + step * W + col) * 4;
+            float yprev = 0.f;
 #pragma unroll
             for (int r = 0; r < 16; ++r) {
               const int rr = (r & 3) + 8 * (r >> 2);
               const float y = fmaxf(acc[i][r] + bv, 0.f) * sc + sh;
-              if constexpr (FULL)
+              if constexpr (PKO) {
+                if (r & 1) {
+                  const unsigned h2 = __builtin_bit_cast(unsigned, __builtin_convertvector(f32x2{yprev, y}, bf16x2));
+                  const f32x2 dl = {yprev - __builtin_bit_cast(float, h2 << 16), y - __builtin_bit_cast(float, h2 & 0xffff0000u)};
+                  const unsigned l2 = __builtin_bit_cast(unsigned, __builtin_convertvector(dl, bf16x2));
+                  const unsigned own = odd ? l2 : h2;
+                  const unsigned got = (unsigned)__builtin_amdgcn_mov_dpp((int)(odd ? h2 : l2), 0xB1, 0xF, 0xF, false);
+                  const unsigned w0 = __builtin_amdgcn_perm(got, own, pk_sel0), w1 = __builtin_amdgcn_perm(got, own, pk_sel1);
+                  const int rp = rr - 1;
+                  if constexpr (FULL) {
+                    __builtin_amdgcn_raw_buffer_store_b32(w0, rout, b0, rp * ldo4, 0);
+                    __builtin_amdgcn_raw_buffer_store_b32(w1, rout, b0, rr * ldo4, 0);
+                  } else {
+                    __builtin_amdgcn_raw_buffer_store_b32(w0, rout, rp >= olo && rp < ohi ? b0 + rp * ldo4 : kOOB, 0, 0);
+                    __builtin_amdgcn_raw_buffer_store_b32(w1, rout, rr >= olo && rr < ohi ? b0 + rr * ldo4 : kOOB, 0, 0);
+                  }
+                }
+                yprev = y;
+              } else if constexpr (FULL) {
                 __builtin_amdgcn_raw_buffer_store_b32(__builtin_bit_cast(unsigned, y), rout, b0, rr * ldo4, 0);
-              else
+              } else {
                 __builtin_amdgcn_raw_buffer_store_b32(__builtin_bit_cast(unsigned, y), rout,
                                                       rr >= olo && rr < ohi ? b0 + rr * ldo4 : kOOB, 0, 0);
+              }
               if constexpr (MODE != 0) {
                 const float x = MODE == 1 ? y + nx[i][r] : nx[i][r];
                 const __bf16 hh = (__bf16)x;
@@ -494,7 +518,10 @@
 template <int W>
 void launch_res2_w(const Res2Args& p, int nblk, hipStream_t s) {
   if (W == 128 && p.variant == 4) {
-    hipLaunchKernelGGL(res2_strip_kernel<4>, dim3(nblk), dim3(256), kSLds, s, p);
+    if (p.out_pk)
+      hipLaunchKernelGGL((res2_strip_kernel<4, true>), dim3(nblk), dim3(256), kSLds, s, p);
+    else
+      hipLaunchKernelGGL((res2_strip_kernel<4, false>), dim3(nblk), dim3(256), kSLds, s, p);
   } else if (p.variant == 3) {
     if constexpr (W == 128) launch_res2_k<W, 128, 4, 8>(p, nblk, s);
     else launch_res2_k<W, 128, 2, 8>(p, nblk, s);
@@ -513,6 +540,8 @@
   WSP_CHECK((long long)p.M * p.ldx * 4 < (long long)kOOB && (long long)p.M * p.ldo * 4 < (long long)kOOB,
             "res2_chain: operand exceeds 2 GiB (split the batch)");
   WSP_CHECK(p.ldx >= 8 * w && p.ldo >= 7 * w && p.ldx % 4 == 0, "res2_chain: bad leading dimensions");
+  WSP_CHECK(!p.out_pk || (w == 128 && p.variant == 4 && p.ldo % 8 == 0),
+            "res2_chain: packed (x3p) output is the strip kernel's (w = 128, variant 4)");
   const int nblk = (p.M + p.rout - 1) / p.rout;
   if (w == 128)
     launch_res2_w<128>(p, nblk, s);
```

After: 26030 (median of 6 runs). Within noise of the previous version (+0.4%).
